# keio-bioinformatics/stem_kernel

Hardware: AMD Instinct MI355X
Metric: sequence-pairs/sec (Gram entries/s) at L=200 nt (higher is better)
Workload: dtype f64

## Files before the change

include/stem_kernel.h:

```cpp
#ifndef STEM_KERNEL_H
#define STEM_KERNEL_H

#include <stddef.h>
#include <stdint.h>

#ifdef __cplusplus
extern "C" {
#endif

#define SK_ABI_VERSION 3

typedef enum {
  SK_OK = 0,
  SK_ERR_INVALID = -1,
  SK_ERR_HIP = -2,
  SK_ERR_NO_DEVICE = -3,
  SK_ERR_ALLOC = -4,
  SK_ERR_RANGE = -5,
  SK_ERR_UNSUPPORTED = -6
} sk_status;

typedef enum {
  SK_SU_STEM = 0,
  SK_SI_STEM = 1,
  SK_SU_STR = 2,
  SK_SI_STR = 3,
  SK_SU_STEM_STR = 4,
  SK_SI_STEM_STR = 5,
  SK_LSU_STEM = 6,
  SK_LSU_STEM_STR = 7,
  SK_NAIVE_STR = 8,
  SK_BPLA = 9,
  SK_LA = 10,
  SK_BPLA_SW = 11,
  SK_LA_SW = 12,
  SK_STEM4D = 13,
  SK_AA_LA = 14,
  SK_AA_LA_SW = 15,
  SK_SIMPAL = 16
} sk_kernel_kind;

typedef struct {
  int32_t kind;
  uint32_t len_band;
  double beta;
  double loop_gap;
  double stack;
  double covar;
  double alpha;
  double gap;
  double match;
  double mismatch;
  double ext;
  double score_table[16];
  double subst;
  double bp_bound;
  int32_t bp_model;
  uint32_t loop;
  double ali_bound;
  int32_t ali_zerop_fixed;
  double aa_score_table[529];
} sk_kernel_params;

void sk_kernel_params_default(sk_kernel_params *p, int32_t kind);

typedef struct sk_context sk_context;

int sk_open(int device, void *hip_stream, sk_context **ctx);
int sk_close(sk_context *ctx);
const char *sk_strerror(int status);
const char *sk_last_error(const sk_context *ctx);

typedef struct sk_dataset sk_dataset;

int sk_dataset_create(sk_dataset **ds);
int sk_dataset_free(sk_dataset *ds);

int sk_dataset_add(sk_dataset *ds, const char *label, int n_rows,
                   const char *const *rows, const double *const *bpp_rows,
                   float th, int use_bp);
int sk_dataset_add_synthetic(sk_dataset *ds, int32_t n, const char *const *seqs,
                             const char *const *labels, float th, int32_t n_threads);
int sk_dataset_add_synthetic_rows(sk_dataset *ds, int32_t n, int32_t n_rows,
                                  const char *const *rows, const char *const *labels,
                                  float th, int32_t n_threads);
int sk_dataset_add_protein(sk_dataset *ds, const char *label, int n_rows,
                           const char *const *rows);
int sk_dataset_aa_profile(const sk_dataset *ds, int i, float *prof24, float *n_seqs);
int sk_char2aa(int c);
int sk_dataset_add_palindromes(sk_dataset *ds, const char *label, const char *seq,
                               const double *bpp, int32_t seed_length, int32_t min_loop,
                               int32_t max_dist);
int sk_dataset_add_palindrome_entries(sk_dataset *ds, const char *label, int32_t seed_length,
                                      int32_t n, const char *keys, const int32_t *dist,
                                      const float *weight);
int sk_dataset_palindromes(const sk_dataset *ds, int i, int32_t *n, char *keys, int32_t *dist,
                           float *weight);
int sk_simpal_shape(int32_t *y_tile, int32_t *x_block);
int sk_dataset_add_copy(sk_dataset *dst, const sk_dataset *src, int32_t i);
int sk_dataset_size(const sk_dataset *ds);
int sk_dataset_export(const sk_dataset *ds, int32_t first, int32_t count, uint8_t *buf,
                      size_t cap, size_t *size);
int sk_dataset_import(sk_dataset *ds, const uint8_t *buf, size_t size);
int sk_dataset_pack_digest(sk_dataset *ds, uint64_t *y_hash, uint64_t *x_hash);
const char *sk_dataset_label(const sk_dataset *ds, int i);
int sk_dataset_shape(const sk_dataset *ds, int i, int32_t *n_nodes,
                     int32_t *n_edges, int32_t *n_bpfreq, int32_t *n_roots,
                     int32_t *seq_len);
int sk_dataset_row_traffic(const sk_dataset *ds, int i, int32_t *rows, int32_t *stored,
                           int32_t *slab_reads, int32_t *gamma_reads, int32_t *phi_reads,
                           int32_t *reg_reads, int32_t *y_slots);
int sk_dataset_dag(const sk_dataset *ds, int i, uint32_t *first, uint32_t *last,
                   uint32_t *n_edges, uint32_t *n_bpfreq, float *weight,
                   uint32_t *max_pa, uint32_t *edge_to, uint32_t *edge_gaps,
                   uint32_t *bp_code, float *bp_p, uint32_t *roots,
                   float *pos_weight);

int sk_dataset_profile(const sk_dataset *ds, int i, float *prof5, float *n_seqs);

int sk_dataset_bpla_weights(const sk_dataset *ds, int i, float *p_left,
                            float *p_right, float *p_unpair);

int sk_dataset_upload(sk_context *ctx, sk_dataset *ds);

int sk_gram(sk_context *ctx, sk_dataset *ds, const sk_kernel_params *kp,
            int normalize, double *out);

int sk_pairs_device(sk_context *ctx, sk_dataset *ds, const sk_kernel_params *kp,
                    const int32_t *x, const int32_t *y, int64_t n_pairs,
                    double *out_dev);
int sk_pairs(sk_context *ctx, sk_dataset *ds, const sk_kernel_params *kp,
             const int32_t *x, const int32_t *y, int64_t n_pairs, double *out);

int sk_test_row(sk_context *ctx, sk_dataset *test, int t, sk_dataset *train,
                const int32_t *sv_index, int32_t n_sv,
                const sk_kernel_params *kp, double *out, double *self);

int sk_diagonal(sk_context *ctx, sk_dataset *ds, const int32_t *sv_index,
                int32_t n_sv, const sk_kernel_params *kp, double *out);

int sk_test_matrix(sk_context *ctx, sk_dataset *test, sk_dataset *train,
                   const sk_kernel_params *kp, int norm_test, int normalize,
                   double *out, double *self_out);

int64_t sk_shard_count(int32_t n, int32_t rank, int32_t world);
int sk_shard_cells(int32_t n, int32_t rank, int32_t world, int32_t *x, int32_t *y);
int sk_shard_assemble(int32_t n, int32_t world, const double *gathered, int64_t per_rank,
                      int normalize, double *out);
int sk_comm_unique_id(uint8_t *id, size_t id_bytes);
int sk_comm_init(sk_context *ctx, const uint8_t *id, size_t id_bytes, int32_t rank, int32_t world);
int sk_comm_allgather(sk_context *ctx, const double *send_dev, int64_t count, double *recv_dev);
int sk_gram_sharded(sk_context *ctx, sk_dataset *ds, const sk_kernel_params *kp, int normalize,
                    double *out);

int sk_format_libsvm(const double *matrix, int32_t rows, int32_t cols,
                     const char *const *labels, char *buf, size_t buf_size,
                     size_t *needed);

int sk_fold_synthetic(const char *seq, int32_t n, int32_t no_gu, double *out);

#define SK_FOLD_NO_GU 1
#define SK_FOLD_NO_CLOSING_GU 2
#define SK_FOLD_NO_LONELY_PAIRS 4
int sk_fold_mccaskill(sk_context *ctx, int32_t n, const char *const *seqs, int32_t flags,
                      double *out, double *log_z);
int sk_fold_sample(sk_context *ctx, int32_t n, const char *const *seqs, int32_t flags,
                   int32_t n_samples, uint64_t seed, double *out_bpp, char *out_structs,
                   double *log_z);
double sk_fold_sample_uniform(uint64_t seed, int32_t seq, int32_t sample, int32_t draw);
int sk_fold_alignment(sk_context *ctx, int32_t n_aln, const int32_t *n_rows,
                      const char *const *rows, int32_t flags, double *out, double *log_z);
int sk_dataset_add_consensus(sk_dataset *ds, const char *label, int n_rows,
                             const char *const *rows, const double *bpp, float th);
int sk_dataset_add_alifolded(sk_context *ctx, sk_dataset *ds, int32_t n, int32_t n_rows,
                             const char *const *rows, const char *const *labels, float th,
                             int32_t fold_flags, int32_t n_threads);
int sk_dataset_add_palindromes_folded(sk_context *ctx, sk_dataset *ds, int32_t n,
                                      const char *const *seqs, const char *const *labels,
                                      int32_t fold_flags, int32_t seed_length, int32_t min_loop,
                                      int32_t max_dist, int32_t n_threads);
int sk_dataset_add_batch(sk_dataset *ds, int32_t n, int32_t n_rows, const char *const *rows,
                         const double *const *bpp_rows, const char *const *labels, float th,
                         int32_t use_bp, int32_t n_threads);
int sk_dataset_add_folded(sk_context *ctx, sk_dataset *ds, int32_t n, int32_t n_rows,
                          const char *const *rows, const char *const *labels, float th,
                          int32_t fold_flags, int32_t n_threads);
int sk_dataset_add_sampled(sk_context *ctx, sk_dataset *ds, int32_t n, int32_t n_rows,
                           const char *const *rows, const char *const *labels, float th,
                           int32_t fold_flags, int32_t n_samples, uint64_t seed, int32_t n_threads);

int sk_bpla_gradients(sk_context *ctx, sk_dataset *xs, sk_dataset *ys, const sk_kernel_params *kp,
                      const int32_t *x, const int32_t *y, int64_t n_pairs, double *value,
                      double *grad);

typedef enum { SK_FMT_FASTA = 0, SK_FMT_CLUSTAL = 1, SK_FMT_MAF = 2 } sk_file_format;
typedef struct sk_seqfile sk_seqfile;
int sk_seqfile_read(const char *path, int32_t format, sk_seqfile **out);
int sk_seqfile_parse(const char *text, size_t len, int32_t format, sk_seqfile **out);
int sk_seqfile_free(sk_seqfile *f);
int64_t sk_seqfile_count(const sk_seqfile *f);
int32_t sk_seqfile_rows(const sk_seqfile *f, int64_t i);
const char *sk_seqfile_row(const sk_seqfile *f, int64_t i, int32_t r);
const char *sk_seqfile_last_error(void);
int sk_random_sequences(uint64_t *state, int32_t n_seqs, int32_t len, char *out);

typedef struct sk_svm_model sk_svm_model;
int sk_svm_model_load(const char *path, sk_svm_model **out);
void sk_svm_model_free(sk_svm_model *m);
int sk_svm_model_info(const sk_svm_model *m, int32_t *svm_type, int32_t *nr_class, int32_t *labels,
                      int32_t *has_probability);
int sk_svm_predict(const sk_svm_model *m, int32_t cnt, const double *row, int32_t n, int32_t probability,
                   double *label, double *values);
const char *sk_svm_last_error(void);

typedef struct {
  const int32_t *train;
  int32_t n_train;
  const int32_t *test;
  int32_t n_test;
  double Cp, Cn, eps;
  int64_t max_iter;
} sk_svm_problem;
typedef enum {
  SK_SVM_CONVERGED = 0,
  SK_SVM_NOT_CONVERGED = 1,
  SK_SVM_NO_PAIR = 2
} sk_svm_status;
typedef struct {
  double rho, obj;
  int64_t iterations;
  int32_t status;
  int32_t n_free;
  int32_t n_bound;
} sk_svm_solution;
int sk_svm_train_batch(sk_context *ctx, const double *gram, int32_t n, const double *labels,
                       const sk_svm_problem *problems, int32_t n_problems, double *alpha_out,
                       double *dec_out, sk_svm_solution *solutions);
int sk_svm_train_batch_host(const double *gram, int32_t n, const double *labels,
                            const sk_svm_problem *problems, int32_t n_problems, int32_t n_threads,
                            double *alpha_out, double *dec_out, sk_svm_solution *solutions);
typedef struct {
  int32_t shrink_calls;
  int32_t shrunk_calls;
  int32_t min_active;
  int32_t unshrunk;
  int32_t regrown;
  int32_t reconstructions;
  int32_t resumed;
} sk_svm_shrink_info;
int sk_svm_train_batch_ex(sk_context *ctx, const double *gram, int32_t n, const double *labels,
                          const sk_svm_problem *problems, int32_t n_problems, int32_t shrinking,
                          double *alpha_out, double *dec_out, sk_svm_solution *solutions,
                          sk_svm_shrink_info *info);
int sk_svm_train_batch_host_ex(const double *gram, int32_t n, const double *labels,
                               const sk_svm_problem *problems, int32_t n_problems, int32_t n_threads,
                               int32_t shrinking, double *alpha_out, double *dec_out,
                               sk_svm_solution *solutions, sk_svm_shrink_info *info);
int sk_svm_train_shape(int32_t *bounds, int32_t *n_classes, int32_t *max_train);
int sk_svm_model_write(const char *path, const double *labels, int32_t n, const int32_t *train,
                       int32_t n_train, const double *alpha, double rho);

typedef enum {
  SK_SVM_C_SVC = 0,
  SK_SVM_NU_SVC = 1,
// ... 102 lines not shown
```

stem_kernel_amd/_lib.py:

```python
from __future__ import annotations

import ctypes as C
import os
import threading

_HERE = os.path.dirname(os.path.abspath(__file__))
LIB_PATH = os.environ.get("SK_LIB_PATH") or os.path.join(_HERE, "libstem_kernel_amd.so")

SK_OK = 0
STATUS = {
    0: "ok", -1: "invalid argument", -2: "HIP runtime error", -3: "no usable gfx950 device",
    -4: "allocation failed", -5: "index out of range", -6: "unsupported",
}

FMT_FASTA, FMT_CLUSTAL, FMT_MAF = range(3)
(SU_STEM, SI_STEM, SU_STR, SI_STR, SU_STEM_STR, SI_STEM_STR, LSU_STEM, LSU_STEM_STR, NAIVE_STR,
 BPLA, LA, BPLA_SW, LA_SW, STEM4D, AA_LA, AA_LA_SW, SIMPAL) = range(17)
AA_LETTERS = "ARNDCQEGHILKMFPSTWYVBZX"


class KernelParams(C.Structure):
    _fields_ = [
        ("kind", C.c_int32), ("len_band", C.c_uint32), ("beta", C.c_double),
        ("loop_gap", C.c_double), ("stack", C.c_double), ("covar", C.c_double),
        ("alpha", C.c_double), ("gap", C.c_double), ("match", C.c_double),
        ("mismatch", C.c_double), ("ext", C.c_double), ("score_table", C.c_double * 16),
        ("subst", C.c_double), ("bp_bound", C.c_double), ("bp_model", C.c_int32),
        ("loop", C.c_uint32), ("ali_bound", C.c_double), ("ali_zerop_fixed", C.c_int32),
        ("aa_score_table", C.c_double * 529),
    ]


class SvmProblem(C.Structure):
    _fields_ = [("train", C.POINTER(C.c_int32)), ("n_train", C.c_int32), ("test", C.POINTER(C.c_int32)),
                ("n_test", C.c_int32), ("Cp", C.c_double), ("Cn", C.c_double), ("eps", C.c_double),
                ("max_iter", C.c_int64)]


class SvmSolution(C.Structure):
    _fields_ = [("rho", C.c_double), ("obj", C.c_double), ("iterations", C.c_int64), ("status", C.c_int32),
                ("n_free", C.c_int32), ("n_bound", C.c_int32)]


class AucProblem(C.Structure):
    _fields_ = [("train", C.POINTER(C.c_int32)), ("n_train", C.c_int32), ("test", C.POINTER(C.c_int32)),
                ("n_test", C.c_int32), ("C", C.c_double), ("alpha", C.POINTER(C.c_double)), ("rho", C.c_double),
                ("delta", C.POINTER(C.c_double))]


class SvmShrinkInfo(C.Structure):
    _fields_ = [(k, C.c_int32) for k in ("shrink_calls", "shrunk_calls", "min_active", "unshrunk", "regrown",
                                         "reconstructions", "resumed")]


class SvmTask(C.Structure):
    _fields_ = [("train", C.POINTER(C.c_int32)), ("n_train", C.c_int32), ("test", C.POINTER(C.c_int32)),
                ("n_test", C.c_int32), ("svm_type", C.c_int32), ("C", C.c_double), ("nu", C.c_double),
                ("p", C.c_double), ("eps", C.c_double), ("max_iter", C.c_int64)]


class SvmTaskSolution(C.Structure):
    _fields_ = [("rho", C.c_double), ("obj", C.c_double), ("iterations", C.c_int64), ("status", C.c_int32),
                ("n_free", C.c_int32), ("n_bound", C.c_int32), ("r", C.c_double)]


class AucInfo(C.Structure):
    _fields_ = [("n_free", C.c_int32), ("n_bound", C.c_int32), ("cg_iterations", C.c_int32),
                ("finite", C.c_int32)]


_P = C.c_void_p
_I32P = C.POINTER(C.c_int32)
_U32P = C.POINTER(C.c_uint32)
_F32P = C.POINTER(C.c_float)
_F64P = C.POINTER(C.c_double)
_I64P = C.POINTER(C.c_int64)

SIGNATURES = {
    "sk_kernel_params_default": (None, [C.POINTER(KernelParams), C.c_int32]),
    "sk_open": (C.c_int, [C.c_int, _P, C.POINTER(_P)]),
    "sk_close": (C.c_int, [_P]),
    "sk_strerror": (C.c_char_p, [C.c_int]),
    "sk_last_error": (C.c_char_p, [_P]),
    "sk_dataset_create": (C.c_int, [C.POINTER(_P)]),
    "sk_dataset_free": (C.c_int, [_P]),
    "sk_dataset_add": (C.c_int, [_P, C.c_char_p, C.c_int, C.POINTER(C.c_char_p),
                                 C.POINTER(_F64P), C.c_float, C.c_int]),
    "sk_dataset_add_synthetic": (C.c_int, [_P, C.c_int32, C.POINTER(C.c_char_p),
                                           C.POINTER(C.c_char_p), C.c_float, C.c_int32]),
    "sk_dataset_add_synthetic_rows": (C.c_int, [_P, C.c_int32, C.c_int32, C.POINTER(C.c_char_p),
                                                C.POINTER(C.c_char_p), C.c_float, C.c_int32]),
    "sk_dataset_add_protein": (C.c_int, [_P, C.c_char_p, C.c_int, C.POINTER(C.c_char_p)]),
    "sk_dataset_aa_profile": (C.c_int, [_P, C.c_int, _F32P, _F32P]),
    "sk_char2aa": (C.c_int, [C.c_int]),
    "sk_last_la_protein": (C.c_int, [_P, C.POINTER(C.c_uint32)]),
    "sk_dataset_add_palindromes": (C.c_int, [_P, C.c_char_p, C.c_char_p, C.POINTER(C.c_double),
                                             C.c_int32, C.c_int32, C.c_int32]),
    "sk_dataset_add_palindromes_folded": (C.c_int, [_P, _P, C.c_int32, C.POINTER(C.c_char_p),
                                                    C.POINTER(C.c_char_p), C.c_int32, C.c_int32,
                                                    C.c_int32, C.c_int32, C.c_int32]),
    "sk_dataset_add_palindrome_entries": (C.c_int, [_P, C.c_char_p, C.c_int32, C.c_int32, C.c_char_p,
                                                    C.POINTER(C.c_int32), _F32P]),
    "sk_dataset_palindromes": (C.c_int, [_P, C.c_int, C.POINTER(C.c_int32), C.c_char_p,
                                         C.POINTER(C.c_int32), _F32P]),
    "sk_simpal_shape": (C.c_int, [C.POINTER(C.c_int32), C.POINTER(C.c_int32)]),
    "sk_dataset_size": (C.c_int, [_P]),
    "sk_dataset_add_copy": (C.c_int, [_P, _P, C.c_int32]),
    "sk_dataset_export": (C.c_int, [_P, C.c_int32, C.c_int32, C.c_void_p, C.c_size_t,
                                    C.POINTER(C.c_size_t)]),
    "sk_dataset_import": (C.c_int, [_P, C.c_void_p, C.c_size_t]),
    "sk_dataset_pack_digest": (C.c_int, [_P, C.POINTER(C.c_uint64), C.POINTER(C.c_uint64)]),
    "sk_dataset_label": (C.c_char_p, [_P, C.c_int]),
    "sk_dataset_shape": (C.c_int, [_P, C.c_int, _I32P, _I32P, _I32P, _I32P, _I32P]),
    "sk_dataset_row_traffic": (C.c_int, [_P, C.c_int, _I32P, _I32P, _I32P, _I32P, _I32P, _I32P, _I32P]),
    "sk_dataset_dag": (C.c_int, [_P, C.c_int, _U32P, _U32P, _U32P, _U32P, _F32P, _U32P,
                                 _U32P, _U32P, _U32P, _F32P, _U32P, _F32P]),
    "sk_dataset_profile": (C.c_int, [_P, C.c_int, _F32P, _F32P]),
    "sk_dataset_bpla_weights": (C.c_int, [_P, C.c_int, _F32P, _F32P, _F32P]),
    "sk_dataset_upload": (C.c_int, [_P, _P]),
    "sk_gram": (C.c_int, [_P, _P, C.POINTER(KernelParams), C.c_int, _F64P]),
    "sk_pairs_device": (C.c_int, [_P, _P, C.POINTER(KernelParams), _I32P, _I32P, C.c_int64,
                                  C.c_void_p]),
    "sk_pairs": (C.c_int, [_P, _P, C.POINTER(KernelParams), _I32P, _I32P, C.c_int64, _F64P]),
    "sk_test_row": (C.c_int, [_P, _P, C.c_int, _P, _I32P, C.c_int32, C.POINTER(KernelParams),
                              _F64P, _F64P]),
    "sk_diagonal": (C.c_int, [_P, _P, _I32P, C.c_int32, C.POINTER(KernelParams), _F64P]),
    "sk_test_matrix": (C.c_int, [_P, _P, _P, C.POINTER(KernelParams), C.c_int, C.c_int, _F64P,
                                 _F64P]),
    "sk_format_libsvm": (C.c_int, [_F64P, C.c_int32, C.c_int32, C.POINTER(C.c_char_p),
                                   C.c_char_p, C.c_size_t, C.POINTER(C.c_size_t)]),
    "sk_fold_synthetic": (C.c_int, [C.c_char_p, C.c_int32, C.c_int32, _F64P]),
    "sk_fold_mccaskill": (C.c_int, [_P, C.c_int32, C.POINTER(C.c_char_p), C.c_int32, _F64P, _F64P]),
    "sk_fold_sample": (C.c_int, [_P, C.c_int32, C.POINTER(C.c_char_p), C.c_int32, C.c_int32, C.c_uint64,
                                 _F64P, C.c_void_p, _F64P]),
    "sk_fold_sample_uniform": (C.c_double, [C.c_uint64, C.c_int32, C.c_int32, C.c_int32]),
    "sk_fold_alignment": (C.c_int, [_P, C.c_int32, _I32P, C.POINTER(C.c_char_p), C.c_int32, _F64P, _F64P]),
    "sk_dataset_add_consensus": (C.c_int, [_P, C.c_char_p, C.c_int, C.POINTER(C.c_char_p), _F64P, C.c_float]),
    "sk_dataset_add_alifolded": (C.c_int, [_P, _P, C.c_int32, C.c_int32, C.POINTER(C.c_char_p),
                                           C.POINTER(C.c_char_p), C.c_float, C.c_int32, C.c_int32]),
    "sk_dataset_add_sampled": (C.c_int, [_P, _P, C.c_int32, C.c_int32, C.POINTER(C.c_char_p),
                                         C.POINTER(C.c_char_p), C.c_float, C.c_int32, C.c_int32,
                                         C.c_uint64, C.c_int32]),
    "sk_dataset_add_batch": (C.c_int, [_P, C.c_int32, C.c_int32, C.POINTER(C.c_char_p),
                                       C.POINTER(_F64P), C.POINTER(C.c_char_p), C.c_float,
                                       C.c_int32, C.c_int32]),
    "sk_dataset_add_folded": (C.c_int, [_P, _P, C.c_int32, C.c_int32, C.POINTER(C.c_char_p),
                                        C.POINTER(C.c_char_p), C.c_float, C.c_int32, C.c_int32]),
    "sk_random_sequences": (C.c_int, [C.POINTER(C.c_uint64), C.c_int32, C.c_int32, C.c_char_p]),
    "sk_last_timing": (C.c_int, [_P, _F64P, _F64P, _F64P, _I32P]),
    "sk_last_launch_ms": (C.c_int, [_P, _F64P, _I32P]),
    "sk_set_async": (C.c_int, [_P, C.c_int32]),
    "sk_sync_timing": (C.c_int, [_P]),
    "sk_shard_count": (C.c_int64, [C.c_int32, C.c_int32, C.c_int32]),
    "sk_shard_cells": (C.c_int, [C.c_int32, C.c_int32, C.c_int32, _I32P, _I32P]),
    "sk_shard_assemble": (C.c_int, [C.c_int32, C.c_int32, _F64P, C.c_int64, C.c_int, _F64P]),
    "sk_comm_unique_id": (C.c_int, [C.c_char_p, C.c_size_t]),
    "sk_comm_init": (C.c_int, [_P, C.c_char_p, C.c_size_t, C.c_int32, C.c_int32]),
    "sk_comm_allgather": (C.c_int, [_P, C.c_void_p, C.c_int64, C.c_void_p]),
    "sk_gram_sharded": (C.c_int, [_P, _P, C.POINTER(KernelParams), C.c_int, _F64P]),
    "sk_last_classes": (C.c_int, [_P, C.POINTER(C.c_uint32), C.POINTER(C.c_uint32)]),
    "sk_last_gamma_shared": (C.c_int32, [_P]),
    "sk_stem4d_col_shape": (C.c_int, [C.c_int32, C.c_int32, _I32P, _I32P, _I32P]),
    "sk_ribosum_tables": (None, [_F32P, _F32P]),
    "sk_char2rna": (C.c_int, [C.c_int]),
    "sk_experiments": (C.c_int, []),
    "sk_bpla_gradients": (C.c_int, [_P, _P, _P, C.POINTER(KernelParams), _I32P, _I32P, C.c_int64,
                                    _F64P, _F64P]),
    "sk_seqfile_read": (C.c_int, [C.c_char_p, C.c_int32, C.POINTER(_P)]),
    "sk_seqfile_parse": (C.c_int, [C.c_char_p, C.c_size_t, C.c_int32, C.POINTER(_P)]),
    "sk_seqfile_free": (C.c_int, [_P]),
    "sk_seqfile_count": (C.c_int64, [_P]),
    "sk_seqfile_rows": (C.c_int32, [_P, C.c_int64]),
    "sk_seqfile_row": (C.c_char_p, [_P, C.c_int64, C.c_int32]),
    "sk_seqfile_last_error": (C.c_char_p, []),
    "sk_svm_model_load": (C.c_int, [C.c_char_p, C.POINTER(_P)]),
    "sk_svm_model_free": (None, [_P]),
    "sk_svm_model_info": (C.c_int, [_P, C.POINTER(C.c_int32), C.POINTER(C.c_int32), C.POINTER(C.c_int32),
                                    C.POINTER(C.c_int32)]),
    "sk_svm_predict": (C.c_int, [_P, C.c_int32, C.POINTER(C.c_double), C.c_int32, C.c_int32,
                                 C.POINTER(C.c_double), C.POINTER(C.c_double)]),
    "sk_svm_last_error": (C.c_char_p, []),
    "sk_svm_train_batch": (C.c_int, [_P, _F64P, C.c_int32, _F64P, C.POINTER(SvmProblem), C.c_int32, _F64P, _F64P,
                                     C.POINTER(SvmSolution)]),
    "sk_svm_train_batch_host": (C.c_int, [_F64P, C.c_int32, _F64P, C.POINTER(SvmProblem), C.c_int32, C.c_int32,
                                          _F64P, _F64P, C.POINTER(SvmSolution)]),
    "sk_svm_train_batch_ex": (C.c_int, [_P, _F64P, C.c_int32, _F64P, C.POINTER(SvmProblem), C.c_int32, C.c_int32,
                                        _F64P, _F64P, C.POINTER(SvmSolution), C.POINTER(SvmShrinkInfo)]),
    "sk_svm_train_batch_host_ex": (C.c_int, [_F64P, C.c_int32, _F64P, C.POINTER(SvmProblem), C.c_int32, C.c_int32,
                                             C.c_int32, _F64P, _F64P, C.POINTER(SvmSolution),
                                             C.POINTER(SvmShrinkInfo)]),
    "sk_svm_train_shape": (C.c_int, [_I32P, _I32P, _I32P]),
    "sk_svm_model_write": (C.c_int, [C.c_char_p, _F64P, C.c_int32, _I32P, C.c_int32, _F64P, C.c_double]),
    "sk_svm_solve_batch": (C.c_int, [_P, _F64P, C.c_int32, _F64P, C.POINTER(SvmTask), C.c_int32, _F64P, _F64P,
                                     C.POINTER(SvmTaskSolution)]),
    "sk_svm_solve_batch_host": (C.c_int, [_F64P, C.c_int32, _F64P, C.POINTER(SvmTask), C.c_int32, C.c_int32,
                                          _F64P, _F64P, C.POINTER(SvmTaskSolution)]),
    "sk_svm_solve_shape": (C.c_int, [_I32P]),
    "sk_svm_model_write_ex": (C.c_int, [C.c_char_p, C.c_int32, _F64P, C.c_int32, _I32P, C.c_int32, _F64P,
                                        C.c_double]),
    "sk_auc_delta": (C.c_int, [_F64P, _F64P, C.c_int32, _F64P, _F64P]),
    "sk_auc_gradient_batch": (C.c_int, [_P, _F64P, _F64P, C.c_int32, C.c_int32, _F64P, C.POINTER(AucProblem),
                                        C.c_int32, _F64P, _F64P, _F64P, C.POINTER(AucInfo)]),
    "sk_auc_gradient_batch_host": (C.c_int, [_F64P, _F64P, C.c_int32, C.c_int32, _F64P, C.POINTER(AucProblem),
                                             C.c_int32, C.c_int32, _F64P, _F64P, _F64P, C.POINTER(AucInfo)]),
    "sk_auc_gradient_shape": (C.c_int, [_I32P, _I32P, C.POINTER(C.c_int64)]),
    "sk_features_create": (C.c_int, [C.c_int32, _I64P, _I32P, _F64P, _I32P, C.POINTER(_P)]),
    "sk_features_parse": (C.c_int, [C.c_char_p, C.c_size_t, C.POINTER(_P)]),
    "sk_features_read": (C.c_int, [C.c_char_p, C.POINTER(_P)]),
    "sk_features_free": (C.c_int, [_P]),
    "sk_features_shape": (C.c_int, [_P, _I32P, _I32P, _I64P]),
    "sk_features_labels": (C.c_int, [_P, _I32P]),
    "sk_features_rows": (C.c_int, [_P, _I64P, _I32P, _F64P]),
    "sk_features_last_error": (C.c_char_p, []),
    "sk_feature_gram_shape": (C.c_int, [_I32P, _I32P, _I32P, _I64P]),
    "sk_feature_dots": (C.c_int, [_P, _P, _P, _F64P]),
    "sk_feature_dots_host": (C.c_int, [_P, _P, C.c_int32, _F64P]),
    "sk_feature_gram": (C.c_int, [_P, _P, C.c_int32, C.c_int32, _F64P, _F64P, _F64P]),
    "sk_feature_gram_host": (C.c_int, [_P, C.c_int32, C.c_int32, _F64P, C.c_int32, _F64P, _F64P]),
    "sk_feature_gram_cross": (C.c_int, [_P, _P, _P, C.c_int32, C.c_int32, _F64P, _F64P]),
    "sk_feature_gram_cross_host": (C.c_int, [_P, _P, C.c_int32, C.c_int32, _F64P, C.c_int32, _F64P]),
}

_lock = threading.Lock()
_lib = None


class StemKernelError(RuntimeError):

    def __init__(self, code, msg=""):
        super().__init__(f"{STATUS.get(code, code)}{': ' + msg if msg else ''}")
        self.code = code


def lib():
    global _lib
    with _lock:
        if _lib is not None:
            return _lib
        if not os.path.exists(LIB_PATH):
            raise StemKernelError(-3, f"{LIB_PATH} not built; run `make` or __graft_entry__.build()")
        try:
            import torch
        except Exception:
            pass
        L = C.CDLL(LIB_PATH)
        for name, (res, args) in SIGNATURES.items():
            f = getattr(L, name)
            f.restype = res
            f.argtypes = args
        _lib = L
        return L


def check(rc, ctx=None):
    if rc != SK_OK:
        msg = ""
        if ctx:
            m = lib().sk_last_error(ctx)
            msg = m.decode() if m else ""
        raise StemKernelError(rc, msg)
    return rc


def default_params(kind=SU_STEM_STR, **over):
    p = KernelParams()
    lib().sk_kernel_params_default(C.byref(p), kind)
    for k, v in over.items():
# ... 8 lines not shown
```

stem_kernel_amd/csrc/host/dataset.cpp:

```cpp
#include <hip/hip_runtime.h>

#include <algorithm>
#include <atomic>
#include <cctype>
#include <chrono>
#include <cmath>
#include <cstdio>
#include <cstdlib>
#include <cstring>
#include <map>
#include <new>
#include <string>
#include <thread>
#include <utility>
#include <vector>

#include "host/runtime_types.h"
#include "blosum62.inc"

namespace sk {
namespace {
int pal_code(char c) {
  switch (c) {
    case 'a': return 0;
// ... 266 lines not shown
    };
    std::vector<Ent> v((size_t)n);
    for (int32_t k = 0; k < n; ++k) {
      uint64_t key = 0;
      for (int t = 0; t < seed_length; ++t) {
        const int c = sk::pal_code(keys[(size_t)k * seed_length + t]);
        if (c < 0) {
          ds->err = "palindrome key letter outside acgu";
          return SK_ERR_INVALID;
        }
        key = (key << 2) | (uint64_t)c;
      }
      if (dist[k] < 0 || !(weight[k] >= 0.0f) || !std::isfinite(weight[k])) {
        ds->err = "palindrome entry with a negative dist or a weight that is not finite and non-negative";
        return SK_ERR_INVALID;
      }
      v[(size_t)k] = Ent{key, dist[k], weight[k]};
    }
    std::sort(v.begin(), v.end(),
              [](const Ent& a, const Ent& b) { return a.key != b.key ? a.key < b.key : a.dist < b.dist; });
    for (size_t k = 1; k < v.size(); ++k)
      if (v[k].key == v[k - 1].key && v[k].dist == v[k - 1].dist) {
        ds->err = "duplicate palindrome entry (key, dist)";
        return SK_ERR_INVALID;
      }
    sk::Example ex;
    ex.pal = true;
    ex.pal_seed = seed_length;
    ex.n_rows = 1;
    ex.n_seqs = 1.0f;
    ex.rows.assign(1, std::string());
    for (const Ent& e : v) {
      ex.pal_key.push_back(e.key);
      ex.pal_dist.push_back(e.dist);
      ex.pal_w.push_back(e.w);
    }
    ds->ex.push_back(std::move(ex));
    ds->labels.emplace_back(label ? label : "");
  } catch (const std::bad_alloc&) {
    return SK_ERR_ALLOC;
  }
  return SK_OK;
}

int sk_dataset_palindromes(const sk_dataset* ds, int i, int32_t* n, char* keys, int32_t* dist, float* weight) {
  if (!ds) return SK_ERR_INVALID;
  if (i < 0 || i >= (int)ds->ex.size()) return SK_ERR_RANGE;
  const sk::Example& X = ds->ex[i];
  if (!X.pal) return SK_ERR_INVALID;
  const size_t m = X.pal_key.size();
  if (n) *n = (int32_t)m;
  if (keys)
    for (size_t k = 0; k < m; ++k)
      for (int t = 0; t < X.pal_seed; ++t)
        keys[k * X.pal_seed + t] = "acgu"[(X.pal_key[k] >> (2 * (X.pal_seed - 1 - t))) & 3];
  if (dist) std::copy(X.pal_dist.begin(), X.pal_dist.end(), dist);
  if (weight) std::copy(X.pal_w.begin(), X.pal_w.end(), weight);
  return SK_OK;
}

int sk_dataset_add_synthetic_rows(sk_dataset* ds, int32_t n, int32_t n_rows,
                                  const char* const* rows, const char* const* labels, float th,
                                  int32_t n_threads) {
  if (!ds || n < 0 || n_rows < 1 || (n > 0 && !rows)) return SK_ERR_INVALID;
  if (ds->uploaded || sk::ds_mixes(ds, sk::kSortRna)) return SK_ERR_INVALID;
  const size_t base = ds->ex.size();
  try {
    ds->ex.resize(base + n);
    for (int32_t i = 0; i < n; ++i) ds->labels.emplace_back(labels && labels[i] ? labels[i] : "+1");
  } catch (const std::bad_alloc&) {
    return SK_ERR_ALLOC;
  }
  int nt = n_threads > 0 ? n_threads : (int)std::thread::hardware_concurrency();
  nt = std::max(1, std::min(nt, std::max<int32_t>(n, 1)));
  std::atomic<int32_t> next(0), status(SK_OK);
  static const bool stats = std::getenv("SK_HOST_STATS") != nullptr;
  std::atomic<int64_t> ns_fold(0), ns_build(0);
  auto work = [&]() {
    std::vector<std::vector<double>> bpp(n_rows);
    std::vector<const double*> bptr(n_rows);
    for (;;) {
      const int32_t i = next.fetch_add(1);
      if (i >= n || status.load() != SK_OK) return;
      try {
        const auto t0 = std::chrono::steady_clock::now();
        const char* const* ex_rows = rows + (size_t)i * n_rows;
        for (int32_t r = 0; r < n_rows; ++r) {
          const char* s = ex_rows[r];
          const int L = (int)std::strlen(s);
          std::string row;
          for (int k = 0; k < L; ++k)
            if (s[k] != '-') row.push_back((char)std::tolower((unsigned char)s[k]));
          bpp[r].assign(row.size() > 1 ? row.size() * (row.size() - 1) / 2 : 1, 0.0);
          sk::fold_nussinov(row.c_str(), (int)row.size(), false, bpp[r].data());
          bptr[r] = bpp[r].data();
        }
        const auto t1 = std::chrono::steady_clock::now();
        sk::build_example(ds->ex[base + i], n_rows, ex_rows, bptr.data(), th, true);
        if (stats) {
          const auto t2 = std::chrono::steady_clock::now();
          ns_fold += std::chrono::duration_cast<std::chrono::nanoseconds>(t1 - t0).count();
          ns_build += std::chrono::duration_cast<std::chrono::nanoseconds>(t2 - t1).count();
        }
      } catch (...) {
        status.store(SK_ERR_INVALID);
      }
    }
  };
  sk::run_pool(nt, work);
  if (stats)
    std::fprintf(stderr, "[sk] synthetic examples: %d on %d threads, fold %.3f s, build %.3f s (thread-seconds)\n", n,
                 nt, ns_fold.load() * 1e-9, ns_build.load() * 1e-9);
  if (status.load() != SK_OK) {
    ds->ex.resize(base);
    ds->labels.resize(base);
  }
  return status.load();
}

int sk_dataset_add_synthetic(sk_dataset* ds, int32_t n, const char* const* seqs,
                             const char* const* labels, float th, int32_t n_threads) {
  return sk_dataset_add_synthetic_rows(ds, n, 1, seqs, labels, th, n_threads);
}

int sk_dataset_size(const sk_dataset* ds) { return ds ? (int)ds->ex.size() : 0; }

const char* sk_dataset_label(const sk_dataset* ds, int i) {
  if (!ds || i < 0 || i >= (int)ds->labels.size()) return nullptr;
  return ds->labels[i].c_str();
}

int sk_dataset_shape(const sk_dataset* ds, int i, int32_t* n_nodes, int32_t* n_edges,
                     int32_t* n_bpfreq, int32_t* n_roots, int32_t* seq_len) {
  if (!ds) return SK_ERR_INVALID;
  if (i < 0 || i >= (int)ds->ex.size()) return SK_ERR_RANGE;
  const sk::Example& X = ds->ex[i];
  if (n_nodes) *n_nodes = X.n_nodes();
  if (n_edges) *n_edges = X.n_edges();
  if (n_bpfreq) *n_bpfreq = (int32_t)X.bpf_code.size();
  if (n_roots) *n_roots = (int32_t)X.roots.size();
  if (seq_len) *seq_len = X.len;
  return SK_OK;
}

int sk_dataset_row_traffic(const sk_dataset* ds, int i, int32_t* rows, int32_t* stored,
                           int32_t* slab_reads, int32_t* gamma_reads, int32_t* phi_reads,
                           int32_t* reg_reads, int32_t* y_slots) {
  if (!ds) return SK_ERR_INVALID;
  if (i < 0 || i >= (int)ds->ex.size()) return SK_ERR_RANGE;
  const sk::HostPack& P = ds->pack;
  if ((int)P.ex_nlxg.size() != (int)ds->ex.size()) return SK_ERR_INVALID;
  int32_t st = 0, sl = 0, ga = 0, ph = 0, rg = 0;
  uint32_t prev = 0xffffu;
  size_t k = (size_t)P.ex_xgch_base[i];
  for (size_t r = (size_t)P.ex_xg_base[i]; r < (size_t)P.ex_xg_base[i] + P.ex_nlxg[i]; ++r) {
    const int ne = P.xgrow[r].a & 0xff;
    for (int t = 0; t < ne; ++t, ++k) {
      const uint32_t c = P.xg_ch[k] & 0xffffu;
      if (c == prev) ++rg;
      else if (c & 0x8000u) ++ga;
      else if (c & 0x4000u) ++ph;
      else ++sl;
    }
    prev = P.xgrow[r].b >> 16;
    st += prev < 0x4000u;
  }
  if (rows) *rows = P.ex_nlxg[i];
  if (stored) *stored = st;
  if (slab_reads) *slab_reads = sl;
  if (gamma_reads) *gamma_reads = ga;
  if (phi_reads) *phi_reads = ph;
  if (reg_reads) *reg_reads = rg;
  if (y_slots) *y_slots = P.ex_nl[i];
  return SK_OK;
}

int sk_dataset_dag(const sk_dataset* ds, int i, uint32_t* first, uint32_t* last,
                   uint32_t* n_edges, uint32_t* n_bpfreq, float* weight, uint32_t* max_pa,
                   uint32_t* edge_to, uint32_t* edge_gaps, uint32_t* bp_code, float* bp_p,
                   uint32_t* roots, float* pos_weight) {
  if (!ds) return SK_ERR_INVALID;
  if (i < 0 || i >= (int)ds->ex.size()) return SK_ERR_RANGE;
  const sk::Example& X = ds->ex[i];
  const int n = X.n_nodes();
  for (int v = 0; v < n; ++v) {
    if (first) first[v] = X.first[v];
    if (last) last[v] = X.last[v];
    if (n_edges) n_edges[v] = X.edge_off[v + 1] - X.edge_off[v];
    if (n_bpfreq) n_bpfreq[v] = X.bpf_off[v + 1] - X.bpf_off[v];
    if (weight) weight[v] = X.weight[v];
    if (max_pa) max_pa[v] = X.max_pa[v];
  }
  if (edge_to) std::copy(X.edge_to.begin(), X.edge_to.end(), edge_to);
  if (edge_gaps) std::copy(X.edge_gaps.begin(), X.edge_gaps.end(), edge_gaps);
  if (bp_code) std::copy(X.bpf_code.begin(), X.bpf_code.end(), bp_code);
  if (bp_p) std::copy(X.bpf_p.begin(), X.bpf_p.end(), bp_p);
  if (roots) std::copy(X.roots.begin(), X.roots.end(), roots);
  if (pos_weight && X.has_bp) std::copy(X.pos_weight.begin(), X.pos_weight.end(), pos_weight);
  return SK_OK;
}

int sk_dataset_profile(const sk_dataset* ds, int i, float* prof5, float* n_seqs) {
  if (!ds) return SK_ERR_INVALID;
  if (i < 0 || i >= (int)ds->ex.size()) return SK_ERR_RANGE;
  const sk::Example& X = ds->ex[i];
  if (prof5) std::copy(X.prof5.begin(), X.prof5.end(), prof5);
  if (n_seqs) *n_seqs = X.n_seqs;
  return SK_OK;
}

int sk_dataset_bpla_weights(const sk_dataset* ds, int i, float* p_left, float* p_right,
                            float* p_unpair) {
  if (!ds) return SK_ERR_INVALID;
  if (i < 0 || i >= (int)ds->ex.size()) return SK_ERR_RANGE;
  const sk::Example& X = ds->ex[i];
  for (int k = 0; k < X.len; ++k) {
    const float4 w = sk::bpla_weight(X, k);
    if (p_left) p_left[k] = w.x;
    if (p_right) p_right[k] = w.y;
    if (p_unpair) p_unpair[k] = w.z;
  }
  return SK_OK;
}

int sk_dataset_add_batch(sk_dataset* ds, int32_t n, int32_t n_rows, const char* const* rows,
                         const double* const* bpp_rows, const char* const* labels, float th,
                         int32_t use_bp, int32_t n_threads) {
  if (!ds || n < 0 || n_rows < 1 || (n > 0 && (!rows || (use_bp && !bpp_rows)))) return SK_ERR_INVALID;
  if (ds->uploaded) return SK_ERR_INVALID;
  return sk::add_examples_threaded(ds, n, n_rows, rows, bpp_rows, labels, th, use_bp, n_threads);
}

}
```

stem_kernel_amd/csrc/host/pack.cpp:

```cpp
#include <hip/hip_runtime.h>

#include <algorithm>
#include <atomic>
#include <chrono>
#include <cmath>
#include <cstdio>
#include <cstdlib>
#include <cstring>
#include <functional>
#include <numeric>
#include <queue>
#include <string>
#include <thread>
#include <type_traits>
#include <utility>
#include <vector>

#include "host/runtime_types.h"

namespace sk {
namespace {

void bpla_weights(const Example& X, std::vector<float4>& out) {
  const int L = X.len;
  const size_t base = out.size();
  out.resize(base + (size_t)std::max(L, 0));
  if (!X.has_bp) {
    for (int i = 0; i < L; ++i) out[base + i] = make_float4(0.f, 0.f, 1.f, 0.f);
    return;
  }
  std::vector<float> pr((size_t)L, 0.0f);
  for (int i = 0; i < L; ++i) {
    float pl = 0.0f;
    if (i + 1 < L) {
      const double* row = X.bpp.data() + sk::tri_index(L, i, i + 1);
      for (int j = i + 1; j < L; ++j) {
        const double b = row[j - i - 1];
        pl = (float)((double)pl + b);
        pr[j] = (float)((double)pr[j] + b);
      }
    }
    float pu = (float)(1.0 - (double)(pl + pr[i]));
    if (pu < 0.0f) pu = 0.0f;
    out[base + i] = make_float4(std::sqrt(pl), std::sqrt(pr[i]), std::sqrt(pu), 0.f);
  }
}

static void pack_palindromes(sk_dataset* ds) {
  sk_dataset::PalPack& P = ds->spack;
  P = sk_dataset::PalPack();
  P.ex_off.push_back(0);
  for (const Example& X : ds->ex) {
    P.key.insert(P.key.end(), X.pal_key.begin(), X.pal_key.end());
    P.dist.insert(P.dist.end(), X.pal_dist.begin(), X.pal_dist.end());
    P.w.insert(P.w.end(), X.pal_w.begin(), X.pal_w.end());
    P.ex_off.push_back((int32_t)P.key.size());
  }
}

static void pack_protein(sk_dataset* ds) {
  sk_dataset::ProtPack& P = ds->ppack;
  P = sk_dataset::ProtPack();
  size_t pos = 0;
  for (const Example& X : ds->ex) pos += (size_t)X.len;
  P.prof.reserve(pos * sk::kAaSlots);
  P.code.reserve(pos);
  for (const Example& X : ds->ex) {
    P.ex_len.push_back(X.len);
    P.ex_pos_base.push_back((int32_t)P.code.size());
    bool coded = true;
    for (int i = 0; i < X.len; ++i) {
      const float* c = X.aa_prof.data() + (size_t)i * sk::kAaSlots;
      int used = 0, slot = sk::kAaSlots - 1;
      for (int k = 0; k < sk::kAaSlots; ++k)
        if (c[k] != 0.0f) {
          ++used;
          slot = k;
        }
      coded = coded && used == 1;
      P.code.push_back((uint8_t)slot);
    }
    if (!coded) std::fill(P.code.end() - X.len, P.code.end(), (uint8_t)(sk::kAaSlots - 1));
    P.ex_coded.push_back(coded ? 1 : 0);
    P.prof.insert(P.prof.end(), X.aa_prof.begin(), X.aa_prof.end());
  }
}

static void assign_sweep_lanes(const std::vector<int>& take, const std::vector<uint32_t>& er, int nl,
                               uint32_t lanes[64]) {
  const int n = (int)take.size();
  thread_local uint8_t npar[2048];
  int cntp[64];
  for (int i = 0; i < n; ++i) ++npar[(er[take[i]] >> 11) & 0x7ff];
  for (int i = 0; i < n; ++i) cntp[i] = npar[(er[take[i]] >> 11) & 0x7ff];
  for (int i = 0; i < n; ++i) npar[(er[take[i]] >> 11) & 0x7ff] = 0;
  int ord[64];
  {
    int cstart[66] = {0};
    for (int i = 0; i < n; ++i) ++cstart[64 - cntp[i] + 1];
    for (int k = 0; k < 65; ++k) cstart[k + 1] += cstart[k];
    for (int i = 0; i < n; ++i) ord[cstart[64 - cntp[i]]++] = i;
  }
  int fill[4] = {0, 0, 0, 0};
  int at[4][16];
  uint32_t rd[2][32][4];
  int rdn[2][32];
  std::memset(at, 0, sizeof(at));
  std::memset(rdn, 0, sizeof(rdn));
  auto child_load = [&](int h, uint32_t c) {
    const int sl = c & 31;
    for (int t = 0; t < std::min(rdn[h][sl], 4); ++t)
      if (rd[h][sl][t] == c) return rdn[h][sl];
    return rdn[h][sl] + 1;
  };
  auto put = [&](int g, uint32_t r) {
    const uint32_t c = r & 0x7ff, q = (r >> 11) & 0x7ff;
    const int h = g >> 1, sl = c & 31;
    bool seen = false;
    for (int t = 0; t < std::min(rdn[h][sl], 4); ++t) seen |= rd[h][sl][t] == c;
    if (!seen) {
      if (rdn[h][sl] < 4) rd[h][sl][rdn[h][sl]] = c;
      ++rdn[h][sl];
    }
    at[g][q & 15]++;
    lanes[16 * g + fill[g]++] = r;
  };
  for (int oi = 0; oi < n; ++oi) {
    const int i = ord[oi];
    const uint32_t r = er[take[i]];
    const uint32_t c = r & 0x7ff, q = (r >> 11) & 0x7ff;
    int best = -1, bc = 1 << 30;
    for (int g = 0; g < 4; ++g) {
      if (fill[g] == 16) continue;
      const int cost = 4 * (child_load(g >> 1, c) + at[g][q & 15] + 1) + fill[g];
      if (cost < bc) {
        bc = cost;
        best = g;
      }
    }
    put(best, r);
  }
  const int nl1 = std::max(nl, 1);
  for (int g = 0; g < 4; ++g) {
    while (fill[g] < 16) {
      int bs = 0, bc = 1 << 30;
      for (int sl = 0; sl < 32 && sl < nl1; ++sl) {
        const int cost = rdn[g >> 1][sl] + at[g][sl & 15];
        if (cost < bc) {
          bc = cost;
          bs = sl;
        }
      }
      const uint32_t d = (uint32_t)(bs % nl1);
      put(g, d | (d << 11));
    }
  }
}

bool is_gamma(const Example& X, int v) {
  const uint32_t e0 = X.edge_off[v], e1 = X.edge_off[v + 1];
  if (e1 - e0 != 1) return false;
  const uint32_t c = X.edge_to[e0];
  if (X.edge_off[c + 1] != X.edge_off[c]) return false;
  return X.bpf_off[v + 1] - X.bpf_off[v] == 1 && X.prof5[(size_t)X.first[v] * 5 + 4] == 0.0f;
}
uint32_t gamma_key(const Example& X, int v) {
  return ((uint32_t)X.bpf_code[X.bpf_off[v]] << 16) | (uint32_t)(X.last[v] - X.first[v]);
}
bool is_phi(const Example& X, int v) {
  const uint32_t e0 = X.edge_off[v], e1 = X.edge_off[v + 1];
  if (e1 == e0 || 2 * (e1 - e0) + 1 > 255) return false;
  if (X.bpf_off[v + 1] - X.bpf_off[v] != 1 || X.prof5[(size_t)X.first[v] * 5 + 4] != 0.0f) return false;
  for (uint32_t k = e0; k < e1; ++k)
    if (!is_gamma(X, X.edge_to[k])) return false;
  return !is_gamma(X, v);
}

struct KeyTables {
  std::vector<uint32_t> gam_key;
  std::vector<uint64_t> phi_raw;
  bool gam_on = false, phi_on = false;
  uint32_t gamma_idx(uint32_t key) const {
    return (uint32_t)(std::lower_bound(gam_key.begin(), gam_key.end(), key) - gam_key.begin());
  }
  uint32_t phi_idx(uint32_t key_p, uint32_t key_c) const {
    const uint64_t k = ((uint64_t)key_c << 32) | key_p;
    return (uint32_t)(std::lower_bound(phi_raw.begin(), phi_raw.end(), k) - phi_raw.begin());
  }
};

KeyTables key_tables(const std::vector<Example>& ex, int nthr) {
  KeyTables K;
  const int n = (int)ex.size();
  {
    std::vector<std::vector<uint32_t>> tk(nthr);
    std::vector<std::vector<uint64_t>> tp(nthr);
    auto keys = [&](int t) {
      for (int e = (int)((int64_t)n * t / nthr); e < (int)((int64_t)n * (t + 1) / nthr); ++e) {
        const Example& X = ex[e];
        for (int v = 0; v < X.n_nodes(); ++v) {
          if (is_gamma(X, v)) tk[t].push_back(gamma_key(X, v));
          if (is_phi(X, v)) {
            tk[t].push_back(gamma_key(X, v));
            for (uint32_t k = X.edge_off[v]; k < X.edge_off[v + 1]; ++k)
              tp[t].push_back(((uint64_t)gamma_key(X, X.edge_to[k]) << 32) | gamma_key(X, v));
          }
        }
        auto& k1 = tk[t];
        if (k1.size() > 4096) {
          std::sort(k1.begin(), k1.end());
          k1.erase(std::unique(k1.begin(), k1.end()), k1.end());
        }
        auto& p1 = tp[t];
        if (p1.size() > 4096) {
          std::sort(p1.begin(), p1.end());
          p1.erase(std::unique(p1.begin(), p1.end()), p1.end());
        }
      }
    };
    run_slices(nthr, keys);
    for (int t = 0; t < nthr; ++t) {
      K.gam_key.insert(K.gam_key.end(), tk[t].begin(), tk[t].end());
      K.phi_raw.insert(K.phi_raw.end(), tp[t].begin(), tp[t].end());
    }
  }
  std::sort(K.gam_key.begin(), K.gam_key.end());
  K.gam_key.erase(std::unique(K.gam_key.begin(), K.gam_key.end()), K.gam_key.end());
  K.gam_on = !K.gam_key.empty() && K.gam_key.size() <= 512 && !SK_KNOB("SK_NO_GAMMA");
  if (!K.gam_on) K.gam_key.clear();
  std::sort(K.phi_raw.begin(), K.phi_raw.end());
  K.phi_raw.erase(std::unique(K.phi_raw.begin(), K.phi_raw.end()), K.phi_raw.end());
  K.phi_on = K.gam_on && !K.phi_raw.empty() && K.phi_raw.size() < 0x4000 && !SK_KNOB("SK_NO_PHI");
  return K;
}

struct YJob {
  int nb0, ebase, bbase, nl;
  bool big;
};
struct YOut {
  std::vector<uint32_t> ysc, ye2, yn_a, yn_b, yn_c;
  std::vector<int32_t> ycs;
  std::vector<uint4> yrec;
  std::vector<float> yn_w, yn_nbp, yn_p0;
  std::vector<double> yn_P;
  int nch = 0;
  std::string err;
};
void pack_y(const HostPack& P, bool sweep_lanes_greedy, const YJob& J, YOut& Y) {
  const int nl = J.nl, ebase = J.ebase, bbase = J.bbase;
  const bool big = J.big;
  {
    std::vector<int> srt(nl);
    std::iota(srt.begin(), srt.end(), 0);
    auto len_of = [&](int k) { return P.nd_b[J.nb0 + k] & 0xffff; };
    std::stable_sort(srt.begin(), srt.end(), [&](int a, int b) { return len_of(a) < len_of(b); });
    std::vector<int> pos(nl);
    for (int i = 0; i < nl; ++i) pos[srt[i]] = i;
    const int nb0 = J.nb0;
    if (big) {
      const int lmax = nl ? (int)(P.nd_b[nb0 + srt[nl - 1]] & 0xffff) : 0;
      for (int v = 0; v <= lmax + 1; ++v) Y.ycs.push_back(0);
      Y.nch = 0;
    } else {
      std::vector<uint32_t> er;
      std::vector<int> epar, ech;
      for (int k = 0; k < nl; ++k) {
        const uint32_t a = P.nd_a[nb0 + k];
        const uint32_t ne = (a >> 16) & 0xff, el = a & 0xffff;
        for (uint32_t t = 0; t < ne; ++t) {
          const uint2 rec = P.ed[ebase + el + t];
          const int c = pos[rec.x & 0xffff], q = pos[k];
          epar.push_back(q);
          ech.push_back(c);
          er.push_back((uint32_t)c | ((uint32_t)q << 11) | ((rec.x >> 16) << 22));
        }
      }
      const int ne_all = (int)er.size();
      std::vector<int> cb(nl + 1, 0), by_child(ne_all);
      for (int f = 0; f < ne_all; ++f) cb[ech[f] + 1]++;
      for (int i = 0; i < nl; ++i) cb[i + 1] += cb[i];
      {
        std::vector<int> fillc(cb.begin(), cb.end() - 1);
        for (int f = 0; f < ne_all; ++f) by_child[fillc[ech[f]]++] = f;
      }
      std::vector<int> h(nl, 0), rem(nl, 0);
      for (int i = nl - 1; i >= 0; --i)
        for (int t = cb[i]; t < cb[i + 1]; ++t) h[i] = std::max(h[i], h[epar[by_child[t]]] + 1);
      for (int f = 0; f < ne_all; ++f) rem[epar[f]]++;
      std::priority_queue<uint64_t, std::vector<uint64_t>, std::greater<uint64_t>> ready;
      auto push_edges_of = [&](int c) {
        const uint64_t len = P.nd_b[nb0 + srt[c]] & 0xffff;
        for (int t = cb[c]; t < cb[c + 1]; ++t) {
          const int f = by_child[t];
          ready.push(((uint64_t)((1 << 20) - 1 - h[epar[f]]) << 44) | (len << 28) | (uint64_t)f);
        }
      };
      for (int c = 0; c < nl; ++c)
        if (rem[c] == 0) push_edges_of(c);
      std::vector<int32_t> cm;
      int32_t run = -1, placed = 0;
      std::vector<int> take, done;
      while (!ready.empty()) {
        take.clear();
        done.clear();
        while (!ready.empty() && (int)take.size() < 64) {
          take.push_back((int)(ready.top() & 0xfffffffu));
          ready.pop();
        }
        for (int f : take) {
          run = std::max<int32_t>(run, (int32_t)(P.nd_b[nb0 + srt[ech[f]]] & 0xffff));
          if (--rem[epar[f]] == 0) done.push_back(epar[f]);
        }
        if (sweep_lanes_greedy) {
          uint32_t lanes[64];
          assign_sweep_lanes(take, er, nl, lanes);
          Y.ysc.insert(Y.ysc.end(), lanes, lanes + 64);
        } else {
          for (int f : take) Y.ysc.push_back(er[f]);
          for (int j = (int)take.size(); j < 64; ++j) {
            const uint32_t d = (uint32_t)(j % std::max(nl, 1));
            Y.ysc.push_back(d | (d << 11));
          }
        }
        placed += (int)take.size();
        cm.push_back(run);
        for (int q : done) push_edges_of(q);
      }
      if (placed != ne_all) {
        Y.err = "IY sweep schedule: DAG has a cycle";
        return;
      }
      const int nch = (int)cm.size();
      const int lmax = nl ? (int)(P.nd_b[nb0 + srt[nl - 1]] & 0xffff) : 0;
      for (int v = 0, c = 0; v <= lmax + 1; ++v) {
        while (c < nch && cm[c] < v) ++c;
        Y.ycs.push_back(c);
      }
      Y.nch = nch;
    }
    const int ye2_base = (int)Y.ye2.size();
    for (int i = 0; i < nl; ++i) {
      const int k = srt[i];
      const uint32_t a = P.nd_a[nb0 + k];
      const uint32_t ne = (a >> 16) & 0xff, el = a & 0xffff;
      const uint32_t nbf = a >> 24, bl = P.nd_b[nb0 + k] >> 16;
      Y.yn_a.push_back(((uint32_t)Y.ye2.size() - ye2_base) | (a & 0xffff0000u));
      for (uint32_t t = 0; t < ne; ++t) {
        const uint2 rec = P.ed[ebase + el + t];
        Y.ye2.push_back(big ? 0u : (uint32_t)pos[rec.x & 0xffff] | ((uint32_t)i << 11) |
                                       ((rec.x >> 16) << 22));
      }
      const bool one = nbf == 1 && P.nd_nbp[nb0 + k] == 0.0f;
      const uint32_t bc0 = nbf ? P.bpf_code[bbase + bl] & 0xf : 0u;
      Y.yn_c.push_back((P.nd_c[nb0 + k] & 0xffff) | (bc0 << 16) | ((one ? 1u : 0u) << 24));
      Y.yn_p0.push_back(nbf ? P.bpf_p[bbase + bl] : 0.0f);
      {
        uint4 r;
        r.x = Y.yn_a.back();
        r.y = Y.yn_c.back();
        std::memcpy(&r.z, &P.nd_w[nb0 + k], 4);
        std::memcpy(&r.w, &Y.yn_p0.back(), 4);
        Y.yrec.push_back(r);
      }
      Y.yn_b.push_back(P.nd_b[nb0 + k]);
      Y.yn_w.push_back(P.nd_w[nb0 + k]);
      Y.yn_nbp.push_back(P.nd_nbp[nb0 + k]);
      Y.yn_P.push_back(P.nd_P[nb0 + k]);
    }
  }
}

struct XOut {
  std::vector<uint32_t> nd_a, nd_b, nd_c, xr_ch, xr_node, gr_info, xg_ch, xg_clg, phk_idx, gra_gidx,
      gra_row, xg_node;
  std::vector<float> nd_w, nd_nbp, bpf_p, gr_pf, xg_cpf, ex_nseqs, pos_w;
  std::vector<double> nd_P, gr_P;
  std::vector<uint2> ed;
  std::vector<uint32_t> bpf_code;
  std::vector<int32_t> lvl, ex_nslots, ex_nlxg, ex_gapless, ex_nl, ex_nlev, ex_len, ex_has_w;
  std::vector<uint8_t> ex_big, xg_cty, pos_chr, ex_dyadic, ex_str_fast, ex_onehot;
  std::vector<sk::XRow> xrow, xgrow;
  std::vector<float4> pos_prof, pos_lru;
  std::vector<uint64_t> ex_phi_bits;
  int nl = 0, nlev = 0, max_slots = 0, n_nostore = 0, n_nodes = 0, gslots = 0;
  bool big = false;
  int rc = SK_OK;
  std::string err;
};
void pack_x(const Example& X, const KeyTables& K, XOut& O) {
  const int nn = X.n_nodes();
  std::vector<int> level(nn, -1);
  int nlev = 0;
  for (int v = 0; v < nn; ++v) {
    const uint32_t e0 = X.edge_off[v], e1 = X.edge_off[v + 1];
    if (e0 == e1) continue;
    int lv = 0;
    bool any_leaf = false;
    for (uint32_t k = e0; k < e1; ++k) {
      const int c = level[X.edge_to[k]];
      if (c < 0) any_leaf = true;
      else lv = std::max(lv, c + 1);
    }
    if (any_leaf && e1 - e0 != 1) {
      O.err = "unexpected DAG shape: stem with a leaf child";
      O.rc = SK_ERR_INVALID;
      return;
    }
    level[v] = lv;
    nlev = std::max(nlev, lv + 1);
  }
  std::vector<int> order;
  {
    std::vector<int> lstart(nlev + 1, 0);
    for (int v = 0; v < nn; ++v)
      if (level[v] >= 0) ++lstart[level[v] + 1];
    for (int l = 0; l < nlev; ++l) lstart[l + 1] += lstart[l];
    order.resize(lstart[nlev]);
    for (int v = 0; v < nn; ++v)
      if (level[v] >= 0) order[lstart[level[v]]++] = v;
  }
  const int nl = (int)order.size();
  if (nl >= 0xffff) {
    O.err = "example too large: more than 65534 non-leaf DAG nodes";
    O.rc = SK_ERR_UNSUPPORTED;
    return;
  }
  std::vector<int> nid(nn, -1);
  for (int k = 0; k < nl; ++k) nid[order[k]] = k;
  std::vector<uint8_t> fl(nn, 0);
  std::vector<uint32_t> gix(nn, 0);
  if (K.gam_on)
    for (int v = 0; v < nn; ++v) fl[v] |= is_gamma(X, v) ? 1 : 0;
  if (K.phi_on)
    for (int v = 0; v < nn; ++v) fl[v] |= is_phi(X, v) ? 2 : 0;
  for (int v = 0; v < nn; ++v)
    if (fl[v]) gix[v] = K.gamma_idx(gamma_key(X, v));
  {
    const size_t ne_x = (size_t)X.n_edges();
    for (auto* q : {&O.nd_a, &O.nd_b, &O.nd_c, &O.xr_node, &O.xg_node}) q->reserve(nl);
    O.nd_w.reserve(nl);
    O.nd_nbp.reserve(nl);
    O.nd_P.reserve(nl);
    O.ed.reserve(ne_x);
    O.xr_ch.reserve(ne_x);
    O.xrow.reserve(nl);
    O.xgrow.reserve(nl);
    O.xg_ch.reserve(2 * ne_x + nl);
    O.xg_clg.reserve(2 * ne_x + nl);
    O.xg_cpf.reserve(2 * ne_x + nl);
    O.xg_cty.reserve(2 * ne_x + nl);
    O.bpf_code.reserve(X.bpf_off[nn]);
    O.bpf_p.reserve(X.bpf_off[nn]);
  }
  std::vector<double> Pw(nn, 0.0);
  for (uint32_t r : X.roots) Pw[r] += 1.0;
  for (int v = nn - 1; v >= 0; --v)
    for (uint32_t k = X.edge_off[v]; k < X.edge_off[v + 1]; ++k) Pw[X.edge_to[k]] += Pw[v];


  bool big_gap = false;
  for (int k = 0; k < nl; ++k) {
    const int v = order[k];
    const uint32_t e0 = X.edge_off[v], e1 = X.edge_off[v + 1];
    const uint32_t b0 = X.bpf_off[v], b1 = X.bpf_off[v + 1];
    const bool loop = level[v] == 0;
    const uint32_t eloc = (uint32_t)O.ed.size(), bloc = (uint32_t)O.bpf_code.size();
    const uint32_t ne = loop ? 0u : e1 - e0;
    if (eloc > 0xffff || bloc > 0xffff || ne > 0xff || b1 - b0 > 0xff ||
        X.last[v] - X.first[v] > 0xffff) {
      O.err = "example too large for the 16-bit packed DAG layout";
      O.rc = SK_ERR_UNSUPPORTED;
      return;
    }
    O.nd_a.push_back(eloc | (ne << 16) | ((b1 - b0) << 24));
    O.nd_b.push_back((X.last[v] - X.first[v]) | (bloc << 16));
    O.nd_c.push_back(loop ? X.edge_gaps[e0] : 0u);
    O.nd_w.push_back(X.weight[v]);
    O.nd_nbp.push_back(X.prof5[(size_t)X.first[v] * 5 + 4]);
    O.nd_P.push_back(Pw[v]);
    if (!loop) {
      for (uint32_t t = e0; t < e1; ++t) {
        const int c = nid[X.edge_to[t]];
        if (c < 0 || X.edge_gaps[t] > 0xffff) {
          O.err = c < 0 ? "unexpected DAG shape: stem with a leaf child" : "gap count exceeds 65535";
          O.rc = c < 0 ? SK_ERR_INVALID : SK_ERR_UNSUPPORTED;
          return;
        }
        big_gap |= X.edge_gaps[t] > 1023;
        O.ed.push_back(make_uint2((uint32_t)c | (X.edge_gaps[t] << 16), (uint32_t)k));
      }
    }
    for (uint32_t t = b0; t < b1; ++t) {
      O.bpf_code.push_back(X.bpf_code[t]);
      O.bpf_p.push_back(X.bpf_p[t]);
    }
  }
  std::vector<int32_t> lv(nlev + 1, 0);
  for (int k = 0; k < nl; ++k) lv[level[order[k]] + 1]++;
  for (int l = 0; l < nlev; ++l) lv[l + 1] += lv[l];
  O.lvl.insert(O.lvl.end(), lv.begin(), lv.end());
  const bool big = nl > 2047 || big_gap;
  O.ex_big.push_back(big ? 1 : 0);

  O.nl = nl;
  O.big = big;

  {
    std::vector<int> last_parent(nn, -1);
    for (int v = 0; v < nn; ++v)
      for (uint32_t k = X.edge_off[v]; k < X.edge_off[v + 1]; ++k)
        last_parent[X.edge_to[k]] = std::max(last_parent[X.edge_to[k]], v);
    std::vector<uint32_t> slot(nn, 0xffff);
    std::vector<int> free_list;
    int nslots = 0;
    for (int v = 0; v < nn; ++v) {
      if (level[v] < 0) continue;
      const bool loop = level[v] == 0;
      const uint32_t e0 = X.edge_off[v], e1 = X.edge_off[v + 1];
      const uint32_t b0 = X.bpf_off[v], b1 = X.bpf_off[v + 1];
      uint32_t nch = 0;
      if (!loop) {
        for (uint32_t k = e0; k < e1; ++k) {
          const int c = X.edge_to[k];
          O.xr_ch.push_back(slot[c] | (X.edge_gaps[k] << 16));
          ++nch;
        }
      }
      for (uint32_t k = e0; k < e1; ++k) {
        const int c = X.edge_to[k];
        if (level[c] >= 0 && last_parent[c] == v && slot[c] != 0xffff) free_list.push_back(slot[c]);
      }
      if (last_parent[v] >= 0) {
        int sl;
        if (!free_list.empty()) {
          sl = free_list.back();
          free_list.pop_back();
        } else {
          sl = nslots++;
        }
        slot[v] = (uint32_t)sl;
      }
      sk::XRow xr;
      xr.a = nch | ((b1 - b0) << 8) | ((loop ? X.edge_gaps[e0] : 0u) << 16);
      xr.b = (X.last[v] - X.first[v]) | (slot[v] << 16);
      xr.w = X.weight[v];
      xr.nbp = X.prof5[(size_t)X.first[v] * 5 + 4];
      xr.bp0 = b1 > b0 ? X.bpf_p[b0] : 0.0f;
      xr.P = Pw[v];
      xr.c = (O.nd_b[nid[v]] >> 16) | ((b1 > b0 ? (uint32_t)X.bpf_code[b0] : 0u) << 16);
      O.xrow.push_back(xr);
      O.xr_node.push_back((uint32_t)nid[v]);
    }
    if (nslots >= 0xffff) {
      O.err = "too many live DAG rows";
      O.rc = SK_ERR_UNSUPPORTED;
      return;
    }
    O.ex_nslots.push_back(nslots);
    O.max_slots = std::max(O.max_slots, nslots);

    std::vector<uint32_t> gslot(nn, 0xffff);
    std::vector<int> gfree;
    int gslots = 0, nlxg = 0;
    std::vector<int> order;
    {
      std::vector<int> npar(nn, 0), cand(nn, -1);
      for (int v = 0; v < nn; ++v)
        for (uint32_t k = X.edge_off[v]; k < X.edge_off[v + 1]; ++k) ++npar[X.edge_to[k]];
      for (int v = 0; v < nn; ++v) {
        if (level[v] <= 0 || (fl[v] & 2)) continue;
        for (uint32_t k = X.edge_off[v]; k < X.edge_off[v + 1] && k < X.edge_off[v] + 4; ++k) {
          const int c = X.edge_to[k];
          if (npar[c] == 1 && level[c] >= 0 && !(fl[c] & 1)) {
            cand[v] = c;
            break;
          }
        }
      }
      if (SK_KNOB("SK_REF_ORDER")) {
        for (int v = 0; v < nn; ++v)
          if (level[v] >= 0) order.push_back(v);
      } else {
        std::vector<uint8_t> seen(nn, 0);
        std::vector<std::pair<int, int>> st;
        auto dfs = [&](int s) {
          if (seen[s] || level[s] < 0) return;
          seen[s] = 1;
          st.push_back({s, 0});
          while (!st.empty()) {
            auto& [v, i] = st.back();
            const int ne = (int)(X.edge_off[v + 1] - X.edge_off[v]);
            int next = -1;
            while (i >= 0 && i < ne && next < 0) {
              const int c = X.edge_to[X.edge_off[v] + i++];
              if (c != cand[v] && !seen[c] && level[c] >= 0) next = c;
            }
            if (next < 0 && i >= 0) {
              i = -1;
              if (cand[v] >= 0 && !seen[cand[v]]) next = cand[v];
            }
            if (next < 0) {
              order.push_back(v);
              st.pop_back();
            } else {
              seen[next] = 1;
              st.push_back({next, 0});
            }
          }
        };
        for (uint32_t r : X.roots) dfs((int)r);
        for (int v = nn - 1; v >= 0; --v) dfs(v);
      }
      std::vector<int> pos(nn, nn), first_parent(nn, nn);
      for (int i = 0; i < (int)order.size(); ++i) pos[order[i]] = i;
      for (int v = 0; v < nn; ++v)
        for (uint32_t k = X.edge_off[v]; k < X.edge_off[v + 1]; ++k) {
          const int c = X.edge_to[k];
          if (pos[v] < nn && (first_parent[c] == nn || pos[v] < pos[first_parent[c]])) first_parent[c] = v;
        }
      const bool move = K.phi_on && !SK_KNOB("SK_PHI_POSTORDER");
      std::vector<int> o1, boff(nn + 2, 0), bl;
      o1.reserve(order.size());
      for (int v : order) {
        if (move && (fl[v] & 2)) ++boff[first_parent[v] + 1];
        else o1.push_back(v);
      }
      for (int i = 0; i <= nn; ++i) boff[i + 1] += boff[i];
      bl.resize(boff[nn + 1]);
      {
        std::vector<int> bf(boff.begin(), boff.end() - 1);
        for (int v : order)
          if (move && (fl[v] & 2)) bl[bf[first_parent[v]]++] = v;
      }
      std::vector<int> o2;
      o2.reserve(order.size() + 8);
      for (int v : o1) {
        const auto bb = bl.begin() + boff[v], be = bl.begin() + boff[v + 1];
        const auto it = std::find(bb, be, cand[v]);
        if (it != be) {
          std::rotate(it, it + 1, be);
          o2.insert(o2.end(), bb, be);
        } else if (bb != be && cand[v] >= 0 && !o2.empty() && o2.back() == cand[v]) {
          o2.pop_back();
          o2.insert(o2.end(), bb, be);
          o2.push_back(cand[v]);
        } else {
          o2.insert(o2.end(), bb, be);
        }
        o2.push_back(v);
      }
      o2.insert(o2.end(), bl.begin() + boff[nn], bl.begin() + boff[nn + 1]);
      order.swap(o2);
    }
    std::vector<int> glast(nn, -1);
    {
      std::vector<int> gpos(nn, -1);
      for (int i = 0; i < (int)order.size(); ++i) gpos[order[i]] = i;
      for (int v : order)
        for (uint32_t k = X.edge_off[v]; k < X.edge_off[v + 1]; ++k) {
          const int c = X.edge_to[k];
          if (glast[c] < 0 || gpos[v] > gpos[glast[c]]) glast[c] = v;
        }
    }
    std::vector<uint8_t> nostore(nn, 0);
    if (!SK_KNOB("SK_STORE_ALL")) {
      std::vector<int> npar(nn, 0), emitted;
      for (int v = 0; v < nn; ++v)
        for (uint32_t k = X.edge_off[v]; k < X.edge_off[v + 1]; ++k) ++npar[X.edge_to[k]];
      for (int v : order)
        if (!(fl[v] & 1)) emitted.push_back(v);
      for (size_t i = 0; i + 1 < emitted.size(); ++i) {
        const int v = emitted[i], r = emitted[i + 1];
        if (npar[v] != 1 || level[r] <= 0 || level[v] < 0 || (fl[r] & 2)) continue;
        for (uint32_t k = X.edge_off[r]; k < X.edge_off[r + 1] && k < X.edge_off[r] + 4; ++k)
          if (X.edge_to[k] == v) nostore[v] = 1;
      }
    }
    for (int v : order) {
      const uint32_t e0 = X.edge_off[v], e1 = X.edge_off[v + 1];
      const uint32_t b0 = X.bpf_off[v], b1 = X.bpf_off[v + 1];
      if (fl[v] & 1) {
        O.gr_info.push_back(gix[v] | (X.edge_gaps[e0] << 16));
        O.gr_pf.push_back(X.bpf_p[b0]);
        O.gr_P.push_back(Pw[v]);
        continue;
      }
      const bool loop = level[v] == 0;
      const bool phi = (fl[v] & 2) != 0;
      uint32_t nch = 0;
      if (phi) {
        const uint32_t kp = gamma_key(X, v);
        for (uint32_t k = e0; k < e1; ++k) {
          const int c = X.edge_to[k];
          const uint32_t kc = gamma_key(X, c);
          const uint32_t pi = K.phi_idx(kp, kc);
          for (int ty : {2, 4}) {
            O.xg_ch.push_back(((ty == 2 ? 0x4000u | pi : 0x8000u | gix[c])) | (X.edge_gaps[k] << 16));
            O.xg_clg.push_back(X.edge_gaps[X.edge_off[c]]);
            O.xg_cpf.push_back(X.bpf_p[X.bpf_off[c]]);
            O.xg_cty.push_back((uint8_t)ty);
          }
          O.phk_idx.push_back(pi);
        }
        O.xg_ch.push_back(0x8000u | gix[v]);
        O.xg_clg.push_back(0u);
        O.xg_cpf.push_back(0.0f);
        O.xg_cty.push_back(3);
        O.gra_gidx.push_back(gix[v]);
        O.gra_row.push_back((uint32_t)O.xgrow.size());
        nch = 2 * (e1 - e0) + 1;
      } else if (!loop) {
        for (uint32_t k = e0; k < e1; ++k) {
          const int c = X.edge_to[k];
          if (fl[c] & 1) {
            O.xg_ch.push_back((0x8000u | gix[c]) | (X.edge_gaps[k] << 16));
            O.xg_clg.push_back(X.edge_gaps[X.edge_off[c]]);
            O.xg_cpf.push_back(X.bpf_p[X.bpf_off[c]]);
            O.xg_cty.push_back(1);
          } else {
            O.xg_ch.push_back(gslot[c] | (X.edge_gaps[k] << 16));
            O.xg_clg.push_back(0u);
            O.xg_cpf.push_back(1.0f);
            O.xg_cty.push_back(0);
          }
          ++nch;
        }
      }
      for (uint32_t k = e0; k < e1; ++k) {
        const int c = X.edge_to[k];
        if (level[c] >= 0 && glast[c] == v && gslot[c] < 0x4000) {
          gfree.push_back(gslot[c]);
          gslot[c] |= 0x10000;
        }
      }
      if (nostore[v]) {
        gslot[v] = 0xfffe;
      } else if (last_parent[v] >= 0) {
        int sl;
        if (!gfree.empty()) {
          sl = gfree.back();
          gfree.pop_back();
        } else {
          sl = gslots++;
        }
        gslot[v] = (uint32_t)sl;
      }
      sk::XRow xr;
      xr.a = nch | ((b1 - b0) << 8) | ((loop ? X.edge_gaps[e0] : 0u) << 16);
      xr.b = (X.last[v] - X.first[v]) | (gslot[v] << 16);
      xr.w = X.weight[v];
      xr.nbp = X.prof5[(size_t)X.first[v] * 5 + 4];
      xr.bp0 = b1 > b0 ? X.bpf_p[b0] : 0.0f;
      xr.P = Pw[v];
      xr.c = (O.nd_b[nid[v]] >> 16) | ((b1 > b0 ? (uint32_t)X.bpf_code[b0] : 0u) << 16) |
             (phi ? 0x80000000u : 0u);
      O.xgrow.push_back(xr);
      O.xg_node.push_back((uint32_t)nid[v]);
      ++nlxg;
    }
    if (K.phi_on) {
      const size_t W = (K.phi_raw.size() + 63) / 64;
      O.ex_phi_bits.assign(W, 0ull);
      for (size_t j = 0; j < O.phk_idx.size(); ++j)
        O.ex_phi_bits[O.phk_idx[j] / 64] |= 1ull << (O.phk_idx[j] % 64);
    }
    if (gslots >= 0x4000) {
      O.err = "too many live DAG rows";
      O.rc = SK_ERR_UNSUPPORTED;
      return;
    }
    O.ex_nlxg.push_back(nlxg);
    O.max_slots = std::max(O.max_slots, gslots);
    O.n_nostore = 0;
    for (int v = 0; v < nn; ++v) O.n_nostore += nostore[v];
    O.n_nodes = nn;
    O.gslots = gslots;
  }
  {
    bool gl = true;
    for (int k = 0; k < nl; ++k) gl &= O.nd_nbp[k] == 0.0f;
    O.ex_gapless.push_back(gl ? 1 : 0);
  }
  O.ex_nl.push_back(nl);
  O.ex_nlev.push_back(nlev);
  O.nlev = nlev;
  O.ex_nseqs.push_back(X.n_seqs);
  O.ex_len.push_back(X.len);
  O.ex_has_w.push_back(X.has_bp ? 1 : 0);
  for (int i = 0; i < X.len; ++i) {
    const float* c = &X.prof5[(size_t)i * 5];
    O.pos_prof.push_back(make_float4(c[0], c[1], c[2], c[3]));
    O.pos_w.push_back(X.has_bp ? X.pos_weight[i] : 1.0f);
    O.pos_chr.push_back((uint8_t)X.rows[0][i]);
  }
  bpla_weights(X, O.pos_lru);
  {
    bool dy = true;
    for (int i = 0; i < X.len; ++i)
      for (int k = 0; k < 4; ++k) {
        const float v = X.prof5[(size_t)i * 5 + k] * 256.0f;
        dy = dy && v == std::rint(v);
      }
    O.ex_dyadic.push_back(dy ? 1 : 0);
    bool full = true;
    for (int i = 0; i < X.len; ++i) {
      const float* c = &X.prof5[(size_t)i * 5];
      full = full && (c[0] + c[1] + c[2] + c[3]) > 0.0f;
    }
    O.ex_str_fast.push_back(dy && full ? 1 : 0);
    bool oh = true;
    for (int i = 0; i < X.len && oh; ++i) {
      const float* c = &X.prof5[(size_t)i * 5];
      int ones = 0, zeros = 0;
      for (int k = 0; k < 4; ++k) {
        ones += c[k] == 1.0f;
        zeros += c[k] == 0.0f;
      }
      oh = ones == 1 && zeros == 3;
    }
    O.ex_onehot.push_back(oh ? 1 : 0);
  }
}

}

float4 bpla_weight(const Example& X, int i) {
  if (!X.has_bp) return make_float4(0.f, 0.f, 1.f, 0.f);
  float pl = 0.0f, pr = 0.0f;
  for (int j = 0; j < i; ++j) pr = (float)((double)pr + X.bpp[sk::tri_index(X.len, j, i)]);
  for (int j = i + 1; j < X.len; ++j) pl = (float)((double)pl + X.bpp[sk::tri_index(X.len, i, j)]);
  float pu = (float)(1.0 - (double)(pl + pr));
  if (pu < 0.0f) pu = 0.0f;
  return make_float4(std::sqrt(pl), std::sqrt(pr), std::sqrt(pu), 0.f);
}

int pack_dataset(sk_dataset* ds, std::string& err, const std::function<void()>* after_x) {
  HostPack& P = ds->pack;
  const bool tstats = std::getenv("SK_HOST_STATS") != nullptr;
  auto tnow = [] { return std::chrono::duration<double, std::milli>(std::chrono::steady_clock::now().time_since_epoch()).count(); };
  const double tp0 = tnow();
  const char* lanes_env = SK_KNOB("SK_SWEEP_LANES");
  const bool sweep_lanes_greedy = !lanes_env || std::atoi(lanes_env) != 0;
  P = HostPack();
  const int n = (int)ds->ex.size();
  const size_t pcap = std::getenv("SK_PACK_THREADS") ? (size_t)std::max(1, std::atoi(std::getenv("SK_PACK_THREADS")))
                                                     : (size_t)16;
  const int nthr = (int)std::max<size_t>(1, std::min<size_t>({(size_t)n / 8 + 1, pcap,
                                                              (size_t)std::max(1u, std::thread::hardware_concurrency())}));
  const KeyTables K = key_tables(ds->ex, nthr);
  P.gam_key = K.gam_key;
  if (K.phi_on)
    for (uint64_t k : K.phi_raw) {
      P.phi_al.push_back((uint32_t)k);
      P.phi_g.push_back(K.gamma_idx((uint32_t)(k >> 32)));
    }
  std::vector<YJob> yjobs;
  yjobs.reserve(n);
  const double tp1 = tnow();
  double tpx = tp1;
  {
    std::vector<XOut> xo(n);
    std::atomic<int> next{0};
    auto work = [&]() {
      for (int e = next.fetch_add(1); e < n; e = next.fetch_add(1)) pack_x(ds->ex[e], K, xo[e]);
    };
    run_pool(nthr, work);
    tpx = tnow();
    P.ex_node_base.push_back(0);
    P.ex_edge_base.push_back(0);
    P.ex_bpf_base.push_back(0);
    P.ex_lvl_base.push_back(0);
    P.ex_pos_base.push_back(0);
#define SK_BIG(X) X(nd_a) X(nd_b) X(nd_c) X(nd_w) X(nd_nbp) X(nd_P) X(ed) X(bpf_code) X(bpf_p) X(lvl) \
  X(xr_ch) X(xrow) X(xr_node) X(gr_info) X(gr_pf) X(gr_P) X(xg_ch) X(xg_clg) X(xg_cpf) X(xg_cty)    \
  X(phk_idx) X(gra_gidx) X(gra_row) X(xgrow) X(xg_node) X(pos_prof) X(pos_w) X(pos_chr) X(pos_lru)  \
  X(ex_phi_bits)
#define SK_OFF(f) std::vector<size_t> off_##f(n + 1, 0);
    SK_BIG(SK_OFF)
#undef SK_OFF
    auto app = [](auto& dst, const auto& src) { dst.insert(dst.end(), src.begin(), src.end()); };
    std::vector<long> st_nodes(n), st_nost(n), st_slots(n);
    for (int e = 0; e < n; ++e) {
      XOut& O = xo[e];
      st_nodes[e] = O.n_nodes;
      st_nost[e] = O.n_nostore;
      st_slots[e] = O.gslots;
      if (O.rc) {
        err = O.err;
        return O.rc;
      }
#define SK_ACC(f) off_##f[e + 1] = off_##f[e] + O.f.size();
      SK_BIG(SK_ACC)
#undef SK_ACC
      yjobs.push_back(YJob{(int)off_nd_a[e], (int)off_ed[e], (int)off_bpf_code[e], O.nl, O.big});
      P.ex_xch_base.push_back((int32_t)off_xr_ch[e]);
      P.ex_xg_base.push_back((int32_t)off_xgrow[e]);
      P.ex_xgch_base.push_back((int32_t)off_xg_ch[e]);
      P.ex_gr_base.push_back((int32_t)off_gr_info[e]);
      P.ex_gra_base.push_back((int32_t)off_gra_gidx[e]);
      P.ex_phk_base.push_back((int32_t)off_phk_idx[e]);
      app(P.ex_big, O.ex_big); app(P.ex_nslots, O.ex_nslots); app(P.ex_nlxg, O.ex_nlxg);
      app(P.ex_gapless, O.ex_gapless); app(P.ex_nl, O.ex_nl); app(P.ex_nlev, O.ex_nlev);
      app(P.ex_nseqs, O.ex_nseqs); app(P.ex_len, O.ex_len); app(P.ex_has_w, O.ex_has_w);
      app(P.ex_dyadic, O.ex_dyadic); app(P.ex_str_fast, O.ex_str_fast); app(P.ex_onehot, O.ex_onehot);
      P.max_slots = std::max(P.max_slots, O.max_slots);
      P.ex_node_base.push_back((int32_t)off_nd_a[e + 1]);
      P.ex_edge_base.push_back((int32_t)off_ed[e + 1]);
      P.ex_bpf_base.push_back((int32_t)off_bpf_code[e + 1]);
      P.ex_lvl_base.push_back((int32_t)off_lvl[e + 1]);
      P.ex_pos_base.push_back((int32_t)off_pos_prof[e + 1]);
      P.max_nl = std::max(P.max_nl, O.nl);
      P.max_edges = std::max(P.max_edges, (int)O.ed.size());
      P.max_bpf = std::max(P.max_bpf, (int)O.bpf_code.size());
      P.max_nlev = std::max(P.max_nlev, O.nlev);
      P.max_len = std::max(P.max_len, ds->ex[e].len);
    }
    const double tq1 = tnow();
#define SK_SIZE(f) P.f.resize(off_##f[n]);
    SK_BIG(SK_SIZE)
#undef SK_SIZE
    const double tq2 = tnow();
    {
      std::atomic<int> nx{0};
      auto copy = [&]() {
        for (int e = nx.fetch_add(1); e < n; e = nx.fetch_add(1)) {
          XOut& O = xo[e];
          for (uint32_t& r : O.gra_row) r += (uint32_t)off_xgrow[e];
#define SK_CPY(f) std::copy(O.f.begin(), O.f.end(), P.f.begin() + off_##f[e]);
          SK_BIG(SK_CPY)
#undef SK_CPY
          O = XOut();
        }
      };
      run_pool(nthr, copy);
    }
    if (tstats) fprintf(stderr, "[sk pack] offsets %.1f ms, resize %.1f ms, copy %.1f ms\n", tq1 - tpx, tq2 - tq1, tnow() - tq2);
#undef SK_BIG
    if (tstats) fprintf(stderr, "[sk pack] keys %.1f ms, x-role %.1f ms (%d threads) + append %.1f ms\n",
                        tp1 - tp0, tpx - tp1, nthr, tnow() - tpx);
    if (std::getenv("SK_PACK_STATS")) {
      long s_rows = 0, s_nost = 0, s_slots = 0, s_nodes = 0, s_st = 0, s_slab = 0, s_gam = 0, s_phi = 0,
           s_reg = 0;
      for (int e = 0; e < n; ++e) {
        s_rows += P.ex_nlxg[e];
        s_nodes += st_nodes[e];
        s_nost += st_nost[e];
        s_slots += st_slots[e];
        uint32_t prev = 0xffffu;
        size_t k = (size_t)P.ex_xgch_base[e];
        for (size_t r = (size_t)P.ex_xg_base[e]; r < (size_t)P.ex_xg_base[e] + P.ex_nlxg[e]; ++r) {
          const int ne = P.xgrow[r].a & 0xff;
          for (int t = 0; t < ne; ++t, ++k) {
            const uint32_t c = P.xg_ch[k] & 0xffffu;
            if (c == prev) ++s_reg;
            else if (c & 0x8000u) ++s_gam;
            else if (c & 0x4000u) ++s_phi;
            else ++s_slab;
          }
          prev = P.xgrow[r].b >> 16;
          s_st += prev < 0x4000u;
        }
      }
      fprintf(stderr,
              "[sk pack] gamma schedule: %ld nodes, %ld rows, %ld unstored, %ld slots; stored %ld, reads: "
              "slab %ld gamma %ld phi %ld, from registers %ld\n",
              s_nodes, s_rows, s_nost, s_slots, s_st, s_slab, s_gam, s_phi, s_reg);
    }
  }
  if (after_x) (*after_x)();
  const double tp2 = tnow();
  {
    std::vector<YOut> yo(yjobs.size());
    const int nthr = (int)std::max<size_t>(1, std::min<size_t>({yjobs.size() / 8 + 1, pcap,
                                                                (size_t)std::max(1u, std::thread::hardware_concurrency())}));
    std::atomic<size_t> next{0};
    auto work = [&]() {
      for (size_t e = next.fetch_add(1); e < yjobs.size(); e = next.fetch_add(1))
        pack_y(P, sweep_lanes_greedy, yjobs[e], yo[e]);
    };
    run_pool(nthr, work);
    const double ty1 = tnow();
    const size_t ny = yo.size();
#define SK_YBIG(X) X(ysc) X(ycs) X(ye2) X(yn_a) X(yn_b) X(yn_c) X(yn_p0) X(yrec) X(yn_w) X(yn_nbp) X(yn_P)
#define SK_OFF(f) std::vector<size_t> off_##f(ny + 1, 0);
    SK_YBIG(SK_OFF)
#undef SK_OFF
    for (size_t e = 0; e < ny; ++e) {
      YOut& Y = yo[e];
      if (!Y.err.empty()) {
        err = Y.err;
        return SK_ERR_INVALID;
      }
#define SK_ACC(f) off_##f[e + 1] = off_##f[e] + Y.f.size();
      SK_YBIG(SK_ACC)
#undef SK_ACC
      P.ex_ysc_base.push_back((int32_t)(off_ysc[e] / 64));
      P.ex_ycs_base.push_back((int32_t)off_ycs[e]);
      P.ex_nch.push_back(Y.nch);
      P.max_nch = std::max(P.max_nch, Y.nch);
    }
#define SK_SIZE(f) P.f.resize(off_##f[ny]);
    SK_YBIG(SK_SIZE)
#undef SK_SIZE
    next = 0;
    auto copy = [&]() {
      for (size_t e = next.fetch_add(1); e < ny; e = next.fetch_add(1)) {
        YOut& Y = yo[e];
#define SK_CPY(f) std::copy(Y.f.begin(), Y.f.end(), P.f.begin() + off_##f[e]);
        SK_YBIG(SK_CPY)
#undef SK_CPY
        Y = YOut();
      }
    };
    run_pool(nthr, copy);
#undef SK_YBIG
    if (tstats) {
      long tch = 0;
      for (int32_t c : P.ex_nch) tch += c;
      fprintf(stderr, "[sk pack] y-role %.1f ms (%d threads) + append %.1f ms; sweep chunks %ld (%.2f per y)\n",
              ty1 - tp2, nthr, tnow() - ty1, tch, P.ex_nch.empty() ? 0.0 : (double)tch / P.ex_nch.size());
    }
  }
  return SK_OK;
}

}

extern "C" {

int sk_dataset_upload(sk_context* ctx, sk_dataset* ds) {
  if (!ctx || !ds) return SK_ERR_INVALID;
  if (ds->uploaded) return ds->device == ctx->device ? SK_OK : sk::fail(ctx, SK_ERR_INVALID, "dataset bound to another device");
  SK_HIP(ctx, hipSetDevice(ctx->device));
  if (sk::ds_pal(ds)) {
    size_t m = 0;
    for (const sk::Example& X : ds->ex) m += X.pal_key.size();
    if (m > (size_t)INT32_MAX) return sk::fail(ctx, SK_ERR_UNSUPPORTED, "palindrome dataset too large");
    try {
      sk::pack_palindromes(ds);
    } catch (const std::bad_alloc&) {
      return sk::fail(ctx, SK_ERR_ALLOC, "palindrome pack");
    }
    const sk_dataset::PalPack& Q = ds->spack;
    SK_HIP(ctx, sk::upload(ds->buf, Q.ex_off, &ds->sdev.ex_off));
    SK_HIP(ctx, sk::upload(ds->buf, Q.key, &ds->sdev.key));
    SK_HIP(ctx, sk::upload(ds->buf, Q.dist, &ds->sdev.dist));
    SK_HIP(ctx, sk::upload(ds->buf, Q.w, &ds->sdev.w));
    ds->spack.key = std::vector<uint64_t>();
    ds->spack.dist = std::vector<int32_t>();
    ds->spack.w = std::vector<float>();
    ds->device = ctx->device;
    ds->uploaded = true;
    return SK_OK;
  }
  if (sk::ds_protein(ds)) {
    size_t pos = 0;
    for (const sk::Example& X : ds->ex) pos += (size_t)X.len;
    if (pos > (size_t)INT32_MAX) return sk::fail(ctx, SK_ERR_UNSUPPORTED, "protein dataset too large");
    try {
      sk::pack_protein(ds);
    } catch (const std::bad_alloc&) {
      return sk::fail(ctx, SK_ERR_ALLOC, "protein pack");
    }
    const sk_dataset::ProtPack& Q = ds->ppack;
    SK_HIP(ctx, sk::upload(ds->buf, Q.ex_len, &ds->pdev.ex_len));
    SK_HIP(ctx, sk::upload(ds->buf, Q.ex_pos_base, &ds->pdev.ex_pos_base));
    SK_HIP(ctx, sk::upload(ds->buf, Q.prof, &ds->pdev.prof));
    SK_HIP(ctx, sk::upload(ds->buf, Q.code, &ds->pdev.code));
    ds->ppack.prof = std::vector<float>();
    ds->ppack.code = std::vector<uint8_t>();
    ds->device = ctx->device;
    ds->uploaded = true;
    return SK_OK;
  }
  std::string err;
  sk::HostPack& P = ds->pack;
  sk::DevSet& D = ds->dev;
  sk::DeviceBuffers& B = ds->buf;
  const bool stats = std::getenv("SK_HOST_STATS") != nullptr;
  const auto tu0 = std::chrono::steady_clock::now();
  std::thread xt;
  hipError_t xe = hipSuccess;
  double x_ms = 0.0;
  auto up_x = [&]() -> hipError_t {
    hipError_t e = hipSetDevice(ctx->device);
    if (e != hipSuccess) return e;
#define SK_UPX(f, d) \
  if ((e = sk::upload(B, P.f, &D.d)) != hipSuccess) return e;
    SK_UPX(ex_nl, ex_nl)
    SK_UPX(ex_node_base, ex_node_base)
    SK_UPX(ex_edge_base, ex_edge_base)
    SK_UPX(ex_bpf_base, ex_bpf_base)
    SK_UPX(ex_lvl_base, ex_lvl_base)
    SK_UPX(ex_nlev, ex_nlev)
    SK_UPX(ex_nseqs, ex_nseqs)
    SK_UPX(ex_len, ex_len)
    SK_UPX(ex_pos_base, ex_pos_base)
    SK_UPX(ex_has_w, ex_has_w)
    SK_UPX(nd_a, nd_a)
    SK_UPX(nd_b, nd_b)
    SK_UPX(nd_c, nd_c)
    SK_UPX(nd_w, nd_w)
    SK_UPX(nd_nbp, nd_nbp)
    SK_UPX(nd_P, nd_P)
    SK_UPX(ed, ed)
    SK_UPX(bpf_code, bpf_code)
    SK_UPX(bpf_p, bpf_p)
    SK_UPX(lvl, lvl)
    SK_UPX(pos_prof, pos_prof)
    SK_UPX(pos_w, pos_w)
    SK_UPX(pos_chr, pos_chr)
    SK_UPX(pos_lru, pos_lru)
    SK_UPX(ex_nslots, ex_nslots)
    SK_UPX(ex_xch_base, ex_xch_base)
    SK_UPX(xrow, xrow)
    SK_UPX(xr_node, xr_node)
    SK_UPX(xr_ch, xr_ch)
    SK_UPX(xgrow, xgrow)
    SK_UPX(xg_node, xg_node)
    SK_UPX(xg_ch, xg_ch)
    SK_UPX(xg_clg, xg_clg)
    SK_UPX(xg_cpf, xg_cpf)
    SK_UPX(ex_xg_base, ex_xg_base)
    SK_UPX(ex_nlxg, ex_nlxg)
    SK_UPX(ex_xgch_base, ex_xgch_base)
    SK_UPX(gr_info, gr_info)
    SK_UPX(gr_pf, gr_pf)
    SK_UPX(gr_P, gr_P)
    SK_UPX(ex_gapless, ex_gapless)
    SK_UPX(gam_key, gam_key)
    SK_UPX(xg_cty, xg_cty)
    SK_UPX(gra_gidx, gra_gidx)
    SK_UPX(gra_row, gra_row)
    SK_UPX(phk_idx, phk_idx)
    SK_UPX(phi_al, phi_al)
    SK_UPX(phi_g, phi_g)
    {
      std::vector<int32_t> grb = P.ex_gr_base;
      grb.push_back((int32_t)P.gr_info.size());
      if ((e = sk::upload(B, grb, &D.ex_gr_base)) != hipSuccess) return e;
      std::vector<int32_t> b1 = P.ex_gra_base, b2 = P.ex_phk_base;
      b1.push_back((int32_t)P.gra_gidx.size());
      b2.push_back((int32_t)P.phk_idx.size());
      if ((e = sk::upload(B, b1, &D.ex_gra_base)) != hipSuccess) return e;
      if ((e = sk::upload(B, b2, &D.ex_phk_base)) != hipSuccess) return e;
    }
#undef SK_UPX
    return hipSuccess;
  };
  const std::function<void()> after_x = [&]() {
    P.xr_ch.insert(P.xr_ch.end(), 8, 0u);
    P.xg_ch.insert(P.xg_ch.end(), 8, 0u);
    auto job = [&]() {
      const auto t0 = std::chrono::steady_clock::now();
      xe = up_x();
      x_ms = std::chrono::duration<double, std::milli>(std::chrono::steady_clock::now() - t0).count();
    };
    try {
      xt = std::thread(job);
    } catch (const std::system_error&) {
      job();
    }
  };
  int rc = sk::pack_dataset(ds, err, &after_x);
  if (xt.joinable()) xt.join();
  if (rc) return sk::fail(ctx, rc, err);
  SK_HIP(ctx, xe);
  const auto tu1 = std::chrono::steady_clock::now();
  D.n_examples = (int32_t)ds->ex.size();
  SK_HIP(ctx, sk::upload(B, P.yn_a, &D.yn_a));
  SK_HIP(ctx, sk::upload(B, P.yn_b, &D.yn_b));
  SK_HIP(ctx, sk::upload(B, P.yn_w, &D.yn_w));
  SK_HIP(ctx, sk::upload(B, P.yn_nbp, &D.yn_nbp));
  SK_HIP(ctx, sk::upload(B, P.yn_P, &D.yn_P));
  SK_HIP(ctx, sk::upload(B, P.ysc, &D.ysc));
  SK_HIP(ctx, sk::upload(B, P.ye2, &D.ye2));
  SK_HIP(ctx, sk::upload(B, P.yn_c, &D.yn_c));
  SK_HIP(ctx, sk::upload(B, P.yn_p0, &D.yn_p0));
  SK_HIP(ctx, sk::upload(B, P.ycs, &D.ycs));
  SK_HIP(ctx, sk::upload(B, P.yrec, &D.yrec));
  SK_HIP(ctx, sk::upload(B, P.ex_ysc_base, &D.ex_ysc_base));
  SK_HIP(ctx, sk::upload(B, P.ex_nch, &D.ex_nch));
  SK_HIP(ctx, sk::upload(B, P.ex_ycs_base, &D.ex_ycs_base));
  D.n_gam = (int32_t)P.gam_key.size();
  D.n_phi = (int32_t)P.phi_al.size();
  D.max_nl = P.max_nl;
  D.max_edges = P.max_edges;
  D.max_bpf = P.max_bpf;
  D.max_nlev = P.max_nlev;
  D.max_nch = P.max_nch;
  D.max_len = P.max_len;
  D.max_slots = P.max_slots;
  D.total_nodes = (int64_t)P.nd_a.size();
  ds->device = ctx->device;
  ds->uploaded = true;
  if (stats) {
    const auto tu2 = std::chrono::steady_clock::now();
    std::fprintf(stderr,
                 "[sk upload] pack + x-role arrays %.1f ms (x-role transfer %.1f ms beside the y-role pack), %zu arrays "
                 "%.1f MB in all, y-role transfer %.1f ms\n",
                 std::chrono::duration<double, std::milli>(tu1 - tu0).count(), x_ms, B.ptrs.size(), B.bytes / 1e6,
                 std::chrono::duration<double, std::milli>(tu2 - tu1).count());
  }
  return SK_OK;
}

int sk_dataset_pack_digest(sk_dataset* ds, uint64_t* y_hash, uint64_t* x_hash) {
  if (!ds || !y_hash || !x_hash) return SK_ERR_INVALID;
  if (ds->uploaded) return SK_ERR_INVALID;
  auto hv = [](const auto& v, uint64_t h) {
    typedef typename std::decay_t<decltype(v)>::value_type T;
    const unsigned char* p = reinterpret_cast<const unsigned char*>(v.data());
    for (size_t i = 0; i < v.size() * sizeof(T); ++i) h = (h ^ p[i]) * 1099511628211ull;
    return h ^ v.size();
  };
  uint64_t hy = 1469598103934665603ull, hx = hy;
  if (sk::ds_pal(ds)) {
    try {
      sk::pack_palindromes(ds);
    } catch (const std::bad_alloc&) {
      return SK_ERR_ALLOC;
    }
    const sk_dataset::PalPack& Q = ds->spack;
    *y_hash = hv(Q.w, hv(Q.dist, hv(Q.key, hy)));
    *x_hash = hv(Q.ex_off, hx);
    ds->spack = sk_dataset::PalPack();
    return SK_OK;
  }
  if (sk::ds_protein(ds)) {
    try {
      sk::pack_protein(ds);
    } catch (const std::bad_alloc&) {
      return SK_ERR_ALLOC;
    }
    const sk_dataset::ProtPack& Q = ds->ppack;
    *y_hash = hv(Q.code, hv(Q.prof, hy));
    *x_hash = hv(Q.ex_coded, hv(Q.ex_pos_base, hv(Q.ex_len, hx)));
    ds->ppack = sk_dataset::ProtPack();
    return SK_OK;
  }
  std::string err;
  const int rc = sk::pack_dataset(ds, err);
  if (rc) return rc;
  const sk::HostPack& P = ds->pack;
#define SK_DG_Y(f) hy = hv(P.f, hy);
#define SK_DG_X(f) hx = hv(P.f, hx);
  SK_PACK_Y_ARRAYS(SK_DG_Y)
  SK_PACK_X_ARRAYS(SK_DG_X)
#undef SK_DG_Y
#undef SK_DG_X
  *y_hash = hy;
  *x_hash = hx;
  ds->pack = sk::HostPack();
  return SK_OK;
}

}
```

stem_kernel_amd/csrc/host/pairs_dag.cpp:

```cpp
#include <hip/hip_runtime.h>

#include <algorithm>
#include <atomic>
#include <chrono>
#include <cmath>
#include <cstdio>
#include <cstdlib>
#include <string>
#include <vector>

#include "host/runtime_types.h"
#include "ribosum85_60.inc"

namespace sk {
namespace {

struct StemClass {
  int maxk = 0;
  int max_nl = 0, max_edges = 0, max_bpf = 0, max_nch = 0;
  int nwaves = 1, grid = 1;
  size_t item_off = 0, n_items = 0;
  size_t slot_off = 0, n_slots = 0;
  bool gam_shared = false;
  bool phi_shared = false;
// ... 226 lines not shown
}

int run_dag_pairs(sk_context* ctx, sk_dataset* xs_, sk_dataset* ys_, const sk_kernel_params* kp,
                      const int32_t* x, const int32_t* y, int64_t n, double* out_dev) {
  int rc = SK_OK;
  const int ny = (int)ys_->ex.size();
  const bool stem = kind_has_stem(kp->kind), str = kind_has_str(kp->kind);
  const HostPack& PX = xs_->pack;
  const HostPack& PY = ys_->pack;
  const bool host_stats = std::getenv("SK_HOST_STATS") != nullptr;
  auto now_ms = [] {
    return std::chrono::duration<double, std::milli>(std::chrono::steady_clock::now().time_since_epoch()).count();
  };
  const double th0 = host_stats ? now_ms() : 0.0;
  double th1 = th0, th2 = th0;

  StemPlan plan;
  const int max_len = std::max(PX.max_len, PY.max_len);
  if (stem) {
    rc = plan_stem_items(ctx, PX, PY, x, y, n, ny, max_len, plan);
    if (rc) return rc;
    ctx->last_cells = plan.cells;
  }

  if (host_stats) th1 = now_ms();
  std::vector<int32_t> item_phi_off, item_phi;
  const bool phi_on = stem && !PX.phi_al.empty() && !PX.gam_key.empty();
  bool two_streams = false;
  double *scratch_cls = nullptr, *scratch_tab = nullptr;
  int64_t big_stride = 0, big_wave = 0;
  int big_grid = 0;
  if (stem) {
    two_streams = plan.classes.size() > 1 && !SK_KNOB("SK_SERIAL_CLASSES");
    size_t scratch_need = 0, scratch_x = 0;
    size_t tab_total = 0;
    size_t phi_budget = SIZE_MAX;
    if (const char* e = SK_KNOB("SK_PHI_TABLE_MB")) phi_budget = (size_t)std::max(0.0, std::atof(e) * 1048576.0);
    auto size_classes = [&](size_t gam_budget) {
      scratch_need = scratch_x = tab_total = 0;
      auto gam_bytes = [&](const StemClass& C) {
        return C.n_slots * (size_t)PX.gam_key.size() * (size_t)(64 * C.maxk + 1) * sizeof(double);
      };
      auto phi_bytes = [&](const StemClass& C) {
        return phi_on ? C.n_slots * (size_t)PX.phi_al.size() * (size_t)(64 * C.maxk + 1) * sizeof(double) : 0;
      };
      size_t total = 0, phi_total = 0;
      for (StemClass& C : plan.classes) {
        C.gam_shared = C.n_slots > 0 && total + gam_bytes(C) <= gam_budget;
        if (C.gam_shared) total += gam_bytes(C);
      }
      for (StemClass& C : plan.classes) {
        C.phi_shared = phi_on && C.gam_shared && total + phi_bytes(C) <= gam_budget &&
                       phi_total + phi_bytes(C) <= phi_budget;
        if (C.phi_shared) {
          total += phi_bytes(C);
          phi_total += phi_bytes(C);
        }
      }
      for (size_t c = 0; c < plan.classes.size(); ++c) {
        StemClass& C = plan.classes[c];
        if (C.gam_shared) {
          C.tab_off = tab_total / sizeof(double);
          tab_total += gam_bytes(C) + (C.phi_shared ? phi_bytes(C) : 0);
        }
        const int64_t slab = (int64_t)(PX.max_slots + 1) * 64 * C.maxk;
        const int64_t gtab1 = (int64_t)PX.gam_key.size() * 64 * C.maxk;
        const int64_t ptab = phi_on ? (int64_t)PX.phi_al.size() * (64 * C.maxk + 1) : 0;
        const size_t b = (size_t)C.grid *
                         (C.nwaves * slab + (C.phi_shared ? 0 : ptab) + (C.gam_shared ? 0 : gtab1)) * sizeof(double);
        size_t& r = (two_streams && (c & 1)) ? scratch_x : scratch_need;
        r = std::max(r, b);
      }
    };
    const bool any_slots = !PX.gam_key.empty() && !plan.slot_y.empty();
    size_classes(any_slots ? SIZE_MAX : 0);
    if (const char* e = SK_KNOB("SK_GAM_TABLE_MB")) {
      size_classes((size_t)std::max(0.0, std::atof(e) * 1048576.0));
    } else if (tab_total > 0 && scratch_need + scratch_x + tab_total + 512 > ctx->scratch_bytes) {
      size_t free_b = 0, total_b = 0;
      SK_HIP(ctx, hipMemGetInfo(&free_b, &total_b));
      size_classes(std::min<size_t>((free_b + ctx->scratch_bytes) / 4, (size_t)8 << 30));
    }
    big_stride = ((int64_t)std::max(plan.big_max_nl, 1) + 63) / 64 * 64;
    big_wave = (int64_t)(PX.max_slots + 2) * big_stride;
    if (!plan.big_x.empty()) {
      size_t free_b = 0, total_b = 0;
      SK_HIP(ctx, hipMemGetInfo(&free_b, &total_b));
      const size_t budget = std::max<size_t>(std::min<size_t>(free_b / 2, (size_t)32 << 30),
                                             (size_t)big_wave * 8 * sk::kStemBigWaves);
      const int64_t by_mem = (int64_t)(budget / ((size_t)big_wave * 8 * sk::kStemBigWaves));
      const int64_t by_pairs = ((int64_t)plan.big_x.size() + sk::kStemBigWaves - 1) / sk::kStemBigWaves;
      big_grid = (int)std::max<int64_t>(1, std::min<int64_t>({by_mem, by_pairs, (int64_t)ctx->n_cu * 8}));
      scratch_need = std::max(scratch_need,
                              (size_t)big_grid * sk::kStemBigWaves * (size_t)big_wave * sizeof(double));
    }
    const size_t big_need = scratch_need;
    auto get_scratch = [&]() {
      scratch_need = (std::max(scratch_need, big_need) + 255) / 256 * 256;
      scratch_x = (scratch_x + 255) / 256 * 256;
      return ensure_scratch(ctx, std::max<size_t>(scratch_need + scratch_x + tab_total, 64));
    };
    rc = get_scratch();
    if (rc && tab_total > 0) {
      (void)hipGetLastError();
      size_classes(0);
      rc = get_scratch();
    }
    if (rc) return rc;
    scratch_cls = ctx->scratch + scratch_need / sizeof(double);
    scratch_tab = scratch_cls + scratch_x / sizeof(double);
  }
  bool phi_items = false;
  for (const StemClass& C : plan.classes) phi_items = phi_items || (phi_on && !C.phi_shared);
  if (phi_items) {
    const size_t W = (PX.phi_al.size() + 63) / 64;
    const size_t ni = plan.items.size();
    std::vector<uint8_t> own(ni, 0);
    for (const StemClass& C : plan.classes)
      if (!C.phi_shared) std::fill(own.begin() + C.item_off, own.begin() + C.item_off + C.n_items, 1);
    const int T = plan_threads((int)(ni / 512 + 1));
    std::vector<std::vector<int32_t>> tkeys(T), tcnt(T);
    run_slices(T, [&](int t) {
      std::vector<uint64_t> acc(W);
      for (size_t i = ni * t / T; i < ni * (t + 1) / T; ++i) {
        const int4 it = plan.items[i];
        const size_t k0 = tkeys[t].size();
        if (own[i] && PY.ex_gapless[it.x]) {
          std::fill(acc.begin(), acc.end(), 0ull);
          for (int u = it.y; u < it.y + it.z; ++u) {
            const uint64_t* b = PX.ex_phi_bits.data() + (size_t)plan.ixs[u] * W;
            for (size_t w = 0; w < W; ++w) acc[w] |= b[w];
          }
          for (size_t w = 0; w < W; ++w)
            for (uint64_t m = acc[w]; m; m &= m - 1) tkeys[t].push_back((int32_t)(w * 64 + __builtin_ctzll(m)));
        }
        tcnt[t].push_back((int32_t)(tkeys[t].size() - k0));
      }
    });
    item_phi_off.assign(1, 0);
    for (int t = 0; t < T; ++t) {
      item_phi.insert(item_phi.end(), tkeys[t].begin(), tkeys[t].end());
      for (int32_t c : tcnt[t]) item_phi_off.push_back(item_phi_off.back() + c);
    }
  }
  if (phi_on && std::getenv("SK_PHI_STATS")) {
    size_t shared = 0, slots = 0;
    for (const StemClass& C : plan.classes) {
      shared += C.phi_shared ? 1 : 0;
      slots += C.phi_shared ? C.n_slots : 0;
    }
    std::fprintf(stderr, "[phi] keys=%zu items=%zu item keys=%zu pairs=%lld phi components=%zu rows=%zu "
                 "classes=%zu sharing=%zu tables=%zu\n",
                 PX.phi_al.size(), plan.items.size(), item_phi.size(), (long long)n, PX.phk_idx.size(),
                 PX.xgrow.size(), plan.classes.size(), shared, slots);
  }

  if (host_stats) th2 = now_ms();
  const StrPlan splan = order_str_pairs(PX, PY, kp, str, x, y, n);
  const size_t n_str_pos = splan.n_sfast ? PX.pos_prof.size() + (ys_ == xs_ ? 0 : PY.pos_prof.size()) : 0;

  const size_t nb = (size_t)n;
  size_t need = 0;
  need += splan.soidx.size() * 8 + n_str_pos * (2 * sizeof(sk::StrPos) + sizeof(sk::StrCode)) + 1024;
  need += (item_phi_off.size() + item_phi.size()) * 4 + 512;
  need += 256 * 8 + 16 * 8 + (size_t)(max_len + 4) * 8 * 2;
  need += 1024 + 256;
  need += plan.items.size() * sizeof(int4) + nb * (4 + 8) + nb * 8 * 2 + nb * 4 * 2 + 64 + 8 * 256;
  need += plan.slot_y.size() * 4 + 256;
  need += plan.big_x.size() * (4 + 4 + 8) + 3 * 256;
  need += 16 * 256;
  rc = ensure_work(ctx, need);
  if (rc) return rc;
  Arena A{static_cast<char*>(ctx->work), 0, ctx->work_bytes};
  double* d_co = A.take<double>(256);
  double* d_gp_loop = A.take<double>(max_len + 4);
  double* d_st = A.take<double>(16);
  double* d_gp_str = A.take<double>(max_len + 4);
  int4* d_items = A.take<int4>(std::max<size_t>(plan.items.size(), 1));
  int32_t* d_ixs = A.take<int32_t>(std::max<size_t>(nb, 1));
  int64_t* d_oidx = A.take<int64_t>(std::max<size_t>(nb, 1));
  double* d_stem = A.take<double>(nb);
  double* d_str = A.take<double>(nb);
  int32_t* d_px = A.take<int32_t>(nb);
  int32_t* d_py = A.take<int32_t>(nb);
  int* d_ctr = A.take<int>(128);
  int32_t* d_sloty = A.take<int32_t>(std::max<size_t>(plan.slot_y.size(), 1));
  int32_t* d_bx = A.take<int32_t>(std::max<size_t>(plan.big_x.size(), 1));
  int32_t* d_by = A.take<int32_t>(std::max<size_t>(plan.big_x.size(), 1));
  int64_t* d_bo = A.take<int64_t>(std::max<size_t>(plan.big_x.size(), 1));
  int32_t* d_iphi_off = A.take<int32_t>(std::max<size_t>(item_phi_off.size(), 1));
  int32_t* d_iphi = A.take<int32_t>(std::max<size_t>(item_phi.size(), 1));
  int64_t* d_soidx = splan.soidx.empty() ? nullptr : A.take<int64_t>(splan.soidx.size());
  sk::StrPos* d_stab = (splan.n_sfast > splan.n_soh) ? A.take<sk::StrPos>(2 * n_str_pos) : nullptr;
  sk::StrCode* d_ctab = splan.n_soh ? A.take<sk::StrCode>(n_str_pos) : nullptr;

  std::vector<double> co(256), st(16);
  const bool subst = kind_subst(kp->kind);
  for (int k = 0; k < 256; ++k)
    co[k] = subst ? std::exp(SK_RIBOSUM_P[k] * kp->beta)
                  : ((k >> 4) == (k & 15) ? kp->stack : kp->covar);
  for (int k = 0; k < 16; ++k)
    st[k] = subst ? std::exp(SK_RIBOSUM_S[k] * kp->alpha)
                  : ((k >> 2) == (k & 3) ? kp->match : kp->mismatch);
  const std::vector<double> gl = gap_powers(kp->loop_gap, max_len + 4);
  const std::vector<double> gs = gap_powers(kp->gap, max_len + 4);
  hipStream_t S = ctx->stream;
  SK_HIP(ctx, sk::h2d(ctx, d_co, co.data(), 256 * 8, S));
  SK_HIP(ctx, sk::h2d(ctx, d_st, st.data(), 16 * 8, S));
  SK_HIP(ctx, sk::h2d(ctx, d_gp_loop, gl.data(), gl.size() * 8, S));
  SK_HIP(ctx, sk::h2d(ctx, d_gp_str, gs.data(), gs.size() * 8, S));
  SK_HIP(ctx, hipMemsetAsync(d_ctr, 0, 128 * sizeof(int), S));

  double* stem_out = (combine_mode(kp->kind) == sk::kCombineStem) ? out_dev : d_stem;
  double* str_out = (combine_mode(kp->kind) == sk::kCombineStr) ? out_dev : d_str;

  const bool side = stem && str;
  if (str) {
    SK_HIP(ctx, sk::h2d(ctx, d_px, splan.spx.empty() ? x : splan.spx.data(), nb * 4, S));
    SK_HIP(ctx, sk::h2d(ctx, d_py, splan.spy.empty() ? y : splan.spy.data(), nb * 4, S));
    if (d_soidx)
      SK_HIP(ctx, sk::h2d(ctx, d_soidx, splan.soidx.data(), splan.soidx.size() * 8, S));
    if (side) {
      SK_HIP(ctx, hipEventRecord(ctx->evf, S));
      SK_HIP(ctx, hipStreamWaitEvent(ctx->side, ctx->evf, 0));
    }
  }
  if (stem) {
    SK_HIP(ctx, sk::h2d(ctx, d_items, plan.items.data(), plan.items.size() * sizeof(int4), S));
    SK_HIP(ctx, sk::h2d(ctx, d_ixs, plan.ixs.data(), nb * 4, S));
    SK_HIP(ctx, sk::h2d(ctx, d_oidx, plan.ioidx.data(), nb * 8, S));
    SK_HIP(ctx, sk::h2d(ctx, d_sloty, plan.slot_y.data(), plan.slot_y.size() * 4, S));
    if (phi_items) {
      SK_HIP(ctx, sk::h2d(ctx, d_iphi_off, item_phi_off.data(), item_phi_off.size() * 4, S));
      if (!item_phi.empty())
        SK_HIP(ctx, sk::h2d(ctx, d_iphi, item_phi.data(), item_phi.size() * 4, S));
    }
    const double gap2 = kp->loop_gap * kp->loop_gap;
    const size_t nnd = std::max<size_t>(PX.nd_a.size(), 1);
    const size_t nxc = std::max<size_t>(PX.xr_ch.size(), 1), nxg = std::max<size_t>(PX.xgrow.size(), 1),
                 nxgc = std::max<size_t>(PX.xg_ch.size(), 1),
                 ngh = std::max<size_t>(PX.ex_nl.size() * PX.gam_key.size(), 1),
                 nphk = std::max<size_t>(PX.phk_idx.size(), 1);
    if (!xs_->prep) {
      void* p = nullptr;
      SK_HIP(ctx, hipMalloc(&p, (3 * nnd + nxc + nxg + nxgc + ngh + nphk) * sizeof(double)));
      xs_->prep = static_cast<double*>(p);
      xs_->buf.ptrs.push_back(p);
      xs_->prep_loop_gap = -1.0;
    }
    sk::DevParamNodes pn;
    pn.nd_L = xs_->prep;
    pn.nd_SL = xs_->prep + nnd;
    pn.xr_SL = xs_->prep + 2 * nnd;
    pn.xr_chw = xs_->prep + 3 * nnd;
    pn.xg_SL = pn.xr_chw + nxc;
    pn.xg_chw = pn.xg_SL + nxg;
    pn.gam_h = pn.xg_chw + nxgc;
    pn.phk_w = pn.gam_h + ngh;
    if (!(xs_->prep_loop_gap == kp->loop_gap)) {
      SK_HIP(ctx, sk::launch_prep(xs_->dev, pn, d_gp_loop, gap2, S));
      xs_->prep_loop_gap = kp->loop_gap;
    }
#ifdef SK_STAMPS
    unsigned long long* d_stamps = nullptr;
    SK_HIP(ctx, hipMalloc(&d_stamps, 16 * sizeof(unsigned long long)));
    SK_HIP(ctx, hipMemsetAsync(d_stamps, 0, 16 * sizeof(unsigned long long), S));
#endif
    if (host_stats)
      std::fprintf(stderr, "[host] pairs=%lld plan %.2f ms, phi keys %.2f ms, uploads+prep %.2f ms\n",
                   (long long)n, th1 - th0, th2 - th1, now_ms() - th2);
    SK_HIP(ctx, hipEventRecord(ctx->ev0, S));
    std::vector<sk::StemLaunch> launches(plan.classes.size());
    for (size_t c = 0; c < plan.classes.size(); ++c) {
      const StemClass& C = plan.classes[c];
      const bool on_cls = two_streams && (c & 1);
      sk::StemLaunch& SL = launches[c];
      SL.xset = xs_->dev;
      SL.yset = ys_->dev;
      SL.pn = pn;
      SL.co_subst = d_co;
      SL.gpow = d_gp_loop;
      SL.n_gpow = max_len + 2;
      SL.n_gpow_pad = (SL.n_gpow + 1) & ~1;
      SL.gap2 = gap2;
      SL.band = kp->len_band;
      SL.lds_max_nl = 64 * C.maxk;
      SL.lds_max_edges = (C.max_edges + 3) & ~3;
      SL.lds_max_bpf = (C.max_bpf + 1 + 3) & ~3;
      SL.lds_max_nch = C.max_nch + 2;
      SL.lds_max_len_pad = (max_len + 2 + 3) & ~3;
      SL.items = d_items + C.item_off;
      SL.n_items = (int32_t)C.n_items;
      SL.xs = d_ixs;
      SL.oidx = d_oidx;
      SL.out = stem_out;
      SL.item_counter = d_ctr + 16 + sk::kStemQueues * (int)c;
      for (int q = 0; q <= sk::kStemQueues; ++q) SL.queue_off[q] = C.queue_off[q];
      SL.slab_doubles = (int64_t)(PX.max_slots + 1) * SL.lds_max_nl;
      SL.scratch = on_cls ? scratch_cls : ctx->scratch;
      SL.gam_on = !PX.gam_key.empty();
      SL.gam_doubles = (int64_t)PX.gam_key.size() * SL.lds_max_nl;
      double* wg_tab = SL.scratch + (size_t)C.grid * C.nwaves * SL.slab_doubles;
      SL.gam_shared = C.gam_shared ? 1 : 0;
      SL.n_slots = C.gam_shared ? (int32_t)C.n_slots : 0;
      SL.slot_y = d_sloty + C.slot_off;
      SL.gam = C.gam_shared ? scratch_tab + C.tab_off : wg_tab;
      SL.kap_y = SL.gam + C.n_slots * (size_t)SL.gam_doubles;
      SL.phi_on = phi_on ? 1 : 0;
      SL.phi_shared = C.phi_shared ? 1 : 0;
      SL.phi_doubles = phi_on ? (int64_t)PX.phi_al.size() * (SL.lds_max_nl + 1) : 0;
      SL.phi = C.phi_shared ? SL.kap_y + C.n_slots * PX.gam_key.size()
                            : wg_tab + (C.gam_shared ? 0 : (size_t)C.grid * SL.gam_doubles);
      SL.item_phi_off = d_iphi_off + (phi_items ? C.item_off : 0);
      SL.item_phi = d_iphi;
#ifdef SK_STAMPS
      SL.stamps = d_stamps;
#endif
    }
    bool any_tables = false;
    for (size_t c = 0; c < plan.classes.size(); ++c) {
      SK_HIP(ctx, sk::launch_gamma_tables(launches[c], plan.classes[c].nwaves, S));
      any_tables = any_tables || plan.classes[c].gam_shared;
    }
    if (two_streams || (side && any_tables)) SK_HIP(ctx, hipEventRecord(ctx->evk, S));
    if (two_streams) SK_HIP(ctx, hipStreamWaitEvent(ctx->cls, ctx->evk, 0));
    if (side && any_tables) SK_HIP(ctx, hipStreamWaitEvent(ctx->side, ctx->evk, 0));
    for (size_t c = 0; c < plan.classes.size(); ++c) {
      const StemClass& C = plan.classes[c];
      const bool on_cls = two_streams && (c & 1);
      const sk::StemLaunch& SL = launches[c];
      SK_HIP(ctx, sk::lev_mark(ctx, on_cls ? ctx->cls : S));
      SK_HIP(ctx, sk::launch_stem(SL, C.grid, C.nwaves, on_cls ? ctx->cls : S));
      SK_HIP(ctx, sk::lev_mark(ctx, on_cls ? ctx->cls : S));
      if (C.gam_shared && (C.phi_shared || !phi_on)) ++ctx->last_gamma_shared;
      ctx->last_stem_classes |= 1u << (C.maxk % 4 ? C.maxk : C.maxk / 4);
    }
    if (two_streams) {
      SK_HIP(ctx, hipEventRecord(ctx->evx, ctx->cls));
      SK_HIP(ctx, hipStreamWaitEvent(S, ctx->evx, 0));
    }
    if (!plan.big_x.empty()) {
      const size_t nbig = plan.big_x.size();
      SK_HIP(ctx, sk::h2d(ctx, d_bx, plan.big_x.data(), nbig * 4, S));
      SK_HIP(ctx, sk::h2d(ctx, d_by, plan.big_y.data(), nbig * 4, S));
      SK_HIP(ctx, sk::h2d(ctx, d_bo, plan.big_o.data(), nbig * 8, S));
      sk::StemBigLaunch BL;
      BL.xset = xs_->dev;
      BL.yset = ys_->dev;
      BL.pn = pn;
      BL.co_subst = d_co;
      BL.gpow = d_gp_loop;
      BL.n_gpow = max_len + 2;
      BL.gap2 = gap2;
      BL.band = kp->len_band;
      BL.xs = d_bx;
      BL.ys = d_by;
      BL.oidx = d_bo;
      BL.n_pairs = (int64_t)nbig;
      BL.out = stem_out;
      BL.scratch = ctx->scratch;
      BL.stride = big_stride;
      BL.wave_doubles = big_wave;
      SK_HIP(ctx, sk::lev_mark(ctx, S));
      SK_HIP(ctx, sk::launch_stem_big(BL, big_grid, S));
      SK_HIP(ctx, sk::lev_mark(ctx, S));
      ctx->last_stem_classes |= 1u;
    }
    SK_HIP(ctx, hipEventRecord(ctx->ev1, S));
#ifdef SK_STAMPS
    {
      unsigned long long h[16];
      SK_HIP(ctx, hipMemcpyAsync(h, d_stamps, sizeof(h), hipMemcpyDeviceToHost, S));
      SK_HIP(ctx, hipStreamSynchronize(S));
      (void)hipFree(d_stamps);
      const double rows = (double)h[8];
      std::fprintf(stderr, "[stamps] classes=%zu pairs=%llu rows=%.0f cycles/row:", plan.classes.size(),
                   h[9], rows);
      const char* nm[7] = {"hdr", "A", "Rfill", "passes", "zero", "sweep", "store"};
      for (int i = 0; i < 7; ++i) std::fprintf(stderr, " %s=%.0f", nm[i], h[i] / rows);
      std::fprintf(stderr, "\n[stamps] per row: A-loaded rows=%.3f swept chunks=%.2f match passes=%.2f band nodes=%.1f\n",
                   h[10] / rows, h[11] / rows, h[12] / rows, h[13] / rows);
      for (const StemClass& C : plan.classes)
        std::fprintf(stderr, "[stamps] class maxk=%d max_nl=%d max_edges=%d max_nch=%d waves/wg=%d grid=%d items=%zu\n",
                     C.maxk, C.max_nl, C.max_edges, C.max_nch, C.nwaves, C.grid, C.n_items);
    }
#endif
    ctx->last_launches = (int32_t)plan.classes.size() + (plan.big_x.empty() ? 0 : 1);
  }
  if (str) {
    const hipStream_t SS = side ? ctx->side : S;
    sk::StrLaunch T;
    T.xset = xs_->dev;
    T.yset = ys_->dev;
// ... 78 lines not shown
```

stem_kernel_amd/csrc/host/runtime_types.h:

```cpp
#pragma once

#include <hip/hip_runtime.h>

#include <algorithm>
#include <cstdint>
#include <cstring>
#include <functional>
#include <memory>
#include <mutex>
#include <new>
#include <string>
#include <system_error>
#include <thread>
#include <utility>
#include <vector>

#include "stem_kernel.h"
#include "host/runtime.h"
#include "host/sk_internal.h"
#include "kernels/device_set.h"
#include "kernels/launch.h"

namespace sk {

struct DeviceBuffers {
  std::vector<void*> ptrs;
  size_t bytes = 0;
  ~DeviceBuffers() { release(); }
  void release() {
    for (void* p : ptrs) (void)hipFree(p);
    ptrs.clear();
  }
};

template <class V, class T = typename V::value_type>
hipError_t upload(DeviceBuffers& db, const V& v, const T** out) {
  void* p = nullptr;
  const size_t bytes = std::max<size_t>(v.size() * sizeof(T), 16);
  hipError_t e = hipMalloc(&p, bytes);
  if (e != hipSuccess) return e;
  db.ptrs.push_back(p);
  db.bytes += bytes;
  if (!v.empty()) e = hipMemcpy(p, v.data(), v.size() * sizeof(T), hipMemcpyHostToDevice);
  *out = static_cast<const T*>(p);
  return e;
}

template <class T>
struct NoInitAlloc : std::allocator<T> {
  template <class U>
  struct rebind {
    using other = NoInitAlloc<U>;
  };
  NoInitAlloc() = default;
  template <class U>
  NoInitAlloc(const NoInitAlloc<U>&) noexcept {}
  template <class U>
  void construct(U* p) noexcept {
    ::new ((void*)p) U;
  }
  template <class U, class... A>
  void construct(U* p, A&&... a) {
    ::new ((void*)p) U(std::forward<A>(a)...);
  }
};
template <class T>
using pvec = std::vector<T, NoInitAlloc<T>>;

struct HostPack {
  std::vector<int32_t> ex_nl, ex_node_base, ex_edge_base, ex_bpf_base, ex_lvl_base, ex_nlev,
      ex_len, ex_pos_base, ex_has_w;
  std::vector<uint8_t> ex_dyadic;
  std::vector<uint8_t> ex_str_fast, ex_onehot;
  std::vector<uint8_t> ex_big;
  std::vector<float> ex_nseqs;
  pvec<uint32_t> nd_a, nd_b, nd_c;
  pvec<float> nd_w, nd_nbp;
  pvec<double> nd_P;
  pvec<uint2> ed;
  pvec<uint32_t> bpf_code;
  pvec<float> bpf_p;
  pvec<int32_t> lvl;
  pvec<float4> pos_prof;
  pvec<float> pos_w;
  pvec<uint8_t> pos_chr;
  pvec<float4> pos_lru;
  std::vector<int32_t> ex_nslots, ex_xch_base;
  pvec<sk::XRow> xrow;
  pvec<uint32_t> yn_a, yn_b, yn_c, ye2, ysc;
  pvec<uint4> yrec;
  pvec<float> yn_w, yn_nbp, yn_p0;
  pvec<double> yn_P;
  pvec<int32_t> ycs;
  std::vector<int32_t> ex_ysc_base, ex_nch, ex_ycs_base;
  pvec<uint32_t> xr_node, xr_ch;
  pvec<sk::XRow> xgrow;
  std::vector<uint32_t> gam_key;
  pvec<uint32_t> xg_node, xg_ch, xg_clg, gr_info;
  pvec<float> xg_cpf, gr_pf;
  pvec<double> gr_P;
  std::vector<int32_t> ex_xg_base, ex_nlxg, ex_xgch_base, ex_gr_base, ex_gapless;
  pvec<uint8_t> xg_cty;
  std::vector<uint32_t> phi_al, phi_g;
  pvec<uint32_t> gra_gidx, gra_row, phk_idx;
  std::vector<int32_t> ex_gra_base, ex_phk_base;
  pvec<uint64_t> ex_phi_bits;
  int32_t max_nl = 0, max_edges = 0, max_bpf = 0, max_nlev = 0, max_len = 0, max_slots = 0;
  int32_t max_nch = 0;
};
#define SK_PACK_Y_ARRAYS(X) X(yn_a) X(yn_b) X(yn_c) X(ye2) X(ysc) X(yrec) X(yn_w) X(yn_nbp) X(yn_p0) X(yn_P) \
  X(ycs) X(ex_ysc_base) X(ex_nch) X(ex_ycs_base)
#define SK_PACK_X_ARRAYS(X) X(nd_a) X(nd_b) X(nd_c) X(nd_w) X(nd_nbp) X(nd_P) X(ed) X(bpf_code) X(bpf_p)     \
  X(lvl) X(xr_ch) X(xrow) X(xr_node) X(gr_info) X(gr_pf) X(gr_P) X(xg_ch) X(xg_clg) X(xg_cpf) X(xg_cty)     \
  X(phk_idx) X(gra_gidx) X(gra_row) X(xgrow) X(xg_node) X(pos_prof) X(pos_w) X(pos_chr) X(pos_lru)          \
  X(ex_phi_bits) X(ex_nl) X(ex_node_base) X(ex_edge_base) X(ex_bpf_base) X(ex_lvl_base) X(ex_nlev) X(ex_len) \
  X(ex_pos_base) X(ex_has_w) X(ex_dyadic) X(ex_str_fast) X(ex_onehot) X(ex_big) X(ex_nseqs) X(ex_nslots)    \
  X(ex_xch_base) X(gam_key) X(ex_xg_base) X(ex_nlxg) X(ex_xgch_base) X(ex_gr_base) X(ex_gapless) X(phi_al)   \
  X(phi_g) X(ex_gra_base) X(ex_phk_base)

struct Stem4dTables {
  Stem4dTables() = default;
  Stem4dTables(const Stem4dTables&) = delete;
  Stem4dTables& operator=(const Stem4dTables&) = delete;
  ~Stem4dTables() {
    if (device < 0 || buf.ptrs.empty()) return;
    int cur = -1;
    if (hipGetDevice(&cur) != hipSuccess) cur = -1;
    if (hipSetDevice(device) == hipSuccess) (void)hipDeviceSynchronize();
    buf.release();
    if (cur >= 0) (void)hipSetDevice(cur);
  }
  DeviceBuffers buf;
  int device = -1, model = -1;
  unsigned loop = 0;
  size_t n_ex = 0;
  const float* bp = nullptr;
  const uint8_t* ch = nullptr;
  std::vector<int64_t> bp_off, ch_off;
  std::vector<uint8_t> why, acgu;
};

}

struct sk_dataset {
  std::vector<sk::Example> ex;
  std::vector<std::string> labels;
  int device = -1;
  bool uploaded = false;
  sk::DevSet dev;
  sk::DeviceBuffers buf;
  sk::HostPack pack;
  struct ProtPack {
    std::vector<int32_t> ex_len, ex_pos_base;
    std::vector<uint8_t> ex_coded, code;
    std::vector<float> prof;
  } ppack;
  sk::LaProtSet pdev;
  struct PalPack {
    std::vector<int32_t> ex_off, dist;
    std::vector<uint64_t> key;
    std::vector<float> w;
  } spack;
  sk::SimpalSet sdev;
  std::string err;
  double* prep = nullptr;
  double prep_loop_gap = -1.0;
  std::mutex s4_mu;
  std::vector<std::shared_ptr<sk::Stem4dTables>> s4;
};

namespace sk {

constexpr size_t kS4Sets = 4;

enum { kSortRna = 0, kSortProtein = 1, kSortPal = 2 };
inline int ex_sort(const Example& X) { return X.pal ? kSortPal : X.protein ? kSortProtein : kSortRna; }
inline bool ds_protein(const sk_dataset* ds) { return !ds->ex.empty() && ds->ex[0].protein; }
inline bool ds_pal(const sk_dataset* ds) { return !ds->ex.empty() && ds->ex[0].pal; }
inline bool ds_mixes(sk_dataset* ds, int sort) {
  if (ds->ex.empty() || ex_sort(ds->ex[0]) == sort) return false;
  static const char* const name[3] = {"RNA", "protein", "palindrome"};
  static const char* const art[3] = {"an", "a", "a"};
  ds->err = std::string(name[sort]) + " example added to " + art[ex_sort(ds->ex[0])] + " " +
            name[ex_sort(ds->ex[0])] + " dataset";
  return true;
}
inline bool pal_seed_differs(sk_dataset* ds, int32_t seed_length) {
  if (!ds_pal(ds) || ds->ex[0].pal_seed == seed_length) return false;
  ds->err = "palindrome example of another seed_length than the dataset's";
  return true;
}
struct Stem4dBatch {
  sk::Stem4dPair* pairs = nullptr;
  int2* items = nullptr;
  int32_t* band = nullptr;
  size_t cap_pairs = 0, cap_items = 0, cap_band = 0;
};

}

struct sk_context {
  sk::Stem4dBatch s4d;
  int device = 0;
  hipStream_t stream = nullptr;
  bool own_stream = false;
  int n_cu = 0;
  std::string err;
  double* scratch = nullptr;
  size_t scratch_bytes = 0;
  void* work = nullptr;
  size_t work_bytes = 0;
  hipEvent_t ev0 = nullptr, ev1 = nullptr, ev2 = nullptr, ev3 = nullptr;
  hipStream_t side = nullptr;
  hipEvent_t evf = nullptr, evj = nullptr;
  hipStream_t cls = nullptr;
  hipEvent_t evk = nullptr, evx = nullptr;
  hipStream_t aux = nullptr;
  hipEvent_t eva = nullptr;
  struct TSet {
    hipEvent_t ev[4] = {nullptr, nullptr, nullptr, nullptr};
    std::vector<hipEvent_t> lev;
    size_t lev_used = 0;
    bool pending = false, stem = false, str = false;
    double cells = 0.0;
    int32_t launches = 0;
  };
  static constexpr int kTSets = 4;
  TSet tset[kTSets];
  int tk = 0;
  bool async = false;
  double acc_stem_ms = 0.0, acc_str_ms = 0.0, acc_cells = 0.0, acc_launch_ms = 0.0;
  int32_t acc_launch_n = 0, acc_launches = 0;
  struct Stage {
    std::vector<std::pair<char*, size_t>> blocks;
    size_t blk = 0, off = 0;
    hipEvent_t ev = nullptr;
    bool recorded = false;
    char* dbuf = nullptr;
    size_t dcap = 0;
    hipEvent_t uev = nullptr;
  };
  Stage stage[2];
  hipStream_t cps = nullptr;
  uint64_t ncalls = 0;
  double last_launch_ms_sum = 0.0;
  int32_t last_launch_n = 0;
  double last_stem_ms = 0.0, last_str_ms = 0.0, last_cells = 0.0;
  int32_t last_launches = 0;
  uint32_t last_stem_classes = 0, last_s4d_classes = 0;
  int32_t last_gamma_shared = 0;
  uint32_t last_la_protein = 0;
  void* comm = nullptr;
};

namespace sk {

template <class F>
void run_slices(int n, F&& f) {
  std::vector<std::thread> th;
  std::vector<int> here;
  for (int t = 1; t < n; ++t) {
    try {
// ... 111 lines not shown
```

stem_kernel_amd/kernel_matrix.py:

```python
from __future__ import annotations

import ctypes as C
import sys
from typing import Iterable, List, Optional, Sequence

import numpy as np

from . import _lib
from ._lib import SK_OK, KernelParams, StemKernelError, check, lib

__all__ = [
    "fold", "random_sequences", "Dataset", "Context", "KernelMatrix",
    "SuStemKernel", "SiStemKernel", "StringKernel", "SuStemStrKernel", "StemStrKernel",
    "SiStemStrKernel", "LSuStemKernel", "LSuStemStrKernel", "NaiveStringKernel",
    "StemKernelError", "SVMModel", "LAKernel", "SimpalKernel", "simpal_shape",
]


_FORMATS = {"fa": _lib.FMT_FASTA, "fasta": _lib.FMT_FASTA, "aln": _lib.FMT_CLUSTAL,
            "clustal": _lib.FMT_CLUSTAL, "maf": _lib.FMT_MAF}


def _seqfile_rows(h) -> List[List[str]]:
    L = lib()
# ... 289 lines not shown
        check(lib().sk_dataset_palindromes(self._h, i, None, kb, d.ctypes.data_as(C.POINTER(C.c_int32)),
                                           w.ctypes.data_as(C.POINTER(C.c_float))))
        raw = kb.raw.rstrip(b"\0")
        s = len(raw) // m if m else 0
        return [raw[k * s:(k + 1) * s].decode() for k in range(m)], d[:m], w[:m]

    def add_file(self, label: str, path: str, fmt: str = "fa", th: float = 0.01,
                 use_bp: bool = True, protein: bool = False) -> int:
        alns = read_examples(path, fmt)
        for rows in alns:
            if protein:
                self.add_protein(label, rows)
            else:
                self.add(label, rows, th=th, use_bp=use_bp)
        return len(alns)

    @classmethod
    def from_sequences(cls, seqs: Iterable[str], labels: Optional[Iterable[str]] = None,
                       th: float = 0.01, bpp: Optional[Sequence[np.ndarray]] = None):
        ds = cls()
        seqs = list(seqs)
        labels = list(labels) if labels is not None else ["+1"] * len(seqs)
        for k, s in enumerate(seqs):
            ds.add(labels[k], [s], None if bpp is None else [bpp[k]], th=th)
        return ds

    @classmethod
    def synthetic(cls, seqs: Sequence[str], labels: Optional[Sequence[str]] = None,
                  th: float = 0.01, threads: int = 0):
        ds = cls()
        n = len(seqs)
        sarr = (C.c_char_p * n)(*[s.encode() for s in seqs])
        larr = None if labels is None else (C.c_char_p * n)(*[l.encode() for l in labels])
        check(lib().sk_dataset_add_synthetic(ds._h, n, sarr, larr, C.c_float(th), threads))
        return ds

    @classmethod
    def synthetic_alignments(cls, alns: Sequence[Sequence[str]], labels=None, th: float = 0.01,
                             threads: int = 0):
        ds = cls()
        n = len(alns)
        nr = len(alns[0]) if n else 1
        if any(len(a) != nr for a in alns):
            raise ValueError("synthetic_alignments needs the same number of rows per alignment")
        flat = [r.encode() for a in alns for r in a]
        rarr = (C.c_char_p * max(len(flat), 1))(*flat)
        larr = None if labels is None else (C.c_char_p * n)(*[l.encode() for l in labels])
        check(lib().sk_dataset_add_synthetic_rows(ds._h, n, nr, rarr, larr, C.c_float(th),
                                                  threads))
        return ds

    def add_batch(self, alns: Sequence[Sequence[str]], bpp_rows=None, labels=None,
                  th: float = 0.01, use_bp: bool = True, threads: int = 0) -> None:
        n = len(alns)
        nr = len(alns[0]) if n else 1
        if any(len(a) != nr for a in alns):
            raise ValueError("add_batch needs the same number of rows per alignment")
        flat = [r.encode() for a in alns for r in a]
        rarr = (C.c_char_p * max(len(flat), 1))(*flat)
        larr = None if labels is None else (C.c_char_p * n)(*[l.encode() for l in labels])
        keep, barr = [], None
        if use_bp:
            barr = (C.POINTER(C.c_double) * max(n * nr, 1))()
            for i in range(n):
                for r in range(nr):
                    b = np.ascontiguousarray(bpp_rows[i][r], dtype=np.float64)
                    if b.size == 0:
                        b = np.zeros(1)
                    keep.append(b)
                    barr[i * nr + r] = b.ctypes.data_as(C.POINTER(C.c_double))
        check(lib().sk_dataset_add_batch(self._h, n, nr, rarr, barr, larr, C.c_float(th),
                                         int(use_bp), threads))

    @classmethod
    def folded(cls, ctx: "Context", alns, labels=None, th: float = 0.01, no_gu: bool = False,
               no_closing_gu: bool = False, threads: int = 0, no_lonely_pairs: bool = False,
               n_samples: int = 0, seed: int = 0, consensus: bool = False):
        alns = [[a] if isinstance(a, str) else list(a) for a in alns]
        ds = cls()
        n = len(alns)
        nr = len(alns[0]) if n else 1
        if any(len(a) != nr for a in alns):
            raise ValueError("folded needs the same number of rows per alignment")
        flat = [r.encode() for a in alns for r in a]
        rarr = (C.c_char_p * max(len(flat), 1))(*flat)
        larr = None if labels is None else (C.c_char_p * n)(*[l.encode() for l in labels])
        flags = (1 if no_gu else 0) | (2 if no_closing_gu else 0) | (4 if no_lonely_pairs else 0)
        if n_samples < 0:
            raise ValueError("n_samples must not be negative")
        if n_samples > 0:
            ctx._chk(lib().sk_dataset_add_sampled(ctx.handle, ds._h, n, nr, rarr, larr, C.c_float(th),
                                                  flags, n_samples, seed, threads))
        elif consensus:
            ctx._chk(lib().sk_dataset_add_alifolded(ctx.handle, ds._h, n, nr, rarr, larr, C.c_float(th),
                                                    flags, threads))
        else:
            ctx._chk(lib().sk_dataset_add_folded(ctx.handle, ds._h, n, nr, rarr, larr, C.c_float(th),
                                                 flags, threads))
        return ds

    def __len__(self):
        return lib().sk_dataset_size(self._h)

    def export(self, first: int = 0, count: Optional[int] = None) -> bytearray:
        count = len(self) - first if count is None else count
        need = C.c_size_t()
        check(lib().sk_dataset_export(self._h, first, count, None, 0, C.byref(need)))
        out = bytearray(need.value)
        buf = (C.c_char * max(need.value, 1)).from_buffer(out) if need.value else None
        check(lib().sk_dataset_export(self._h, first, count, buf, need.value, C.byref(need)))
        return out

    def import_bytes(self, data) -> "Dataset":
        n = len(data)
        if isinstance(data, bytearray) and n:
            data = (C.c_char * n).from_buffer(data)
        check(lib().sk_dataset_import(self._h, data, n))
        return self

    def pack_digest(self):
        hy, hx = C.c_uint64(), C.c_uint64()
        check(lib().sk_dataset_pack_digest(self._h, C.byref(hy), C.byref(hx)))
        return hy.value, hx.value

    def profile(self, i: int):
        L = self.shape(i)[4]
        out = np.zeros((max(L, 1), 5), np.float32)
        ns = C.c_float()
        check(lib().sk_dataset_profile(self._h, i, out.ctypes.data_as(C.POINTER(C.c_float)),
                                       C.byref(ns)))
        return out[:L], ns.value

    def bpla_weights(self, i: int):
        L = self.shape(i)[4]
        a = [np.zeros(max(L, 1), np.float32) for _ in range(3)]
        check(lib().sk_dataset_bpla_weights(self._h, i, *(v.ctypes.data_as(C.POINTER(C.c_float))
                                                           for v in a)))
        return [v[:L] for v in a]

    def label(self, i: int) -> str:
        return lib().sk_dataset_label(self._h, i).decode()

    def shape(self, i: int):
        v = [C.c_int32() for _ in range(5)]
        check(lib().sk_dataset_shape(self._h, i, *[C.byref(a) for a in v]))
        return tuple(a.value for a in v)

    def row_traffic(self, i: int) -> dict:
        v = [C.c_int32() for _ in range(7)]
        check(lib().sk_dataset_row_traffic(self._h, i, *[C.byref(a) for a in v]))
        return dict(zip(("rows", "stored", "slab_reads", "gamma_reads", "phi_reads", "reg_reads",
                         "y_slots"), (a.value for a in v)))

    def dag(self, i: int) -> dict:
        nn, ne, nb, nr, L = self.shape(i)
        u = lambda k: np.zeros(max(k, 1), np.uint32)
        f = lambda k: np.zeros(max(k, 1), np.float32)
        d = dict(first=u(nn), last=u(nn), n_edges=u(nn), n_bpfreq=u(nn), weight=f(nn),
                 max_pa=u(nn), edge_to=u(ne), edge_gaps=u(ne), bp_code=u(nb), bp_p=f(nb),
                 roots=u(nr), pos_weight=f(L))
        ptr = lambda a: a.ctypes.data_as(C.POINTER(C.c_uint32 if a.dtype == np.uint32 else C.c_float))
        check(lib().sk_dataset_dag(self._h, i, *[ptr(d[k]) for k in
                                                 ("first", "last", "n_edges", "n_bpfreq", "weight",
                                                  "max_pa", "edge_to", "edge_gaps", "bp_code",
                                                  "bp_p", "roots", "pos_weight")]))
        sizes = dict(first=nn, last=nn, n_edges=nn, n_bpfreq=nn, weight=nn, max_pa=nn,
                     edge_to=ne, edge_gaps=ne, bp_code=nb, bp_p=nb, roots=nr, pos_weight=L)
        return {k: v[: sizes[k]] for k, v in d.items()}


class Context:

    def __init__(self, device: int = 0, stream: Optional[int] = None):
        self._h = C.c_void_p()
        check(lib().sk_open(device, C.c_void_p(stream) if stream else None, C.byref(self._h)))
        self.device = device

    def close(self):
        if self._h is not None and self._h.value:
            lib().sk_close(self._h)
            self._h = None

    def __del__(self):
        try:
            self.close()
        except Exception:
            pass

    @property
    def handle(self):
        return self._h

    def _chk(self, rc):
        return check(rc, self._h)

    def fold(self, seqs: Sequence[str], no_gu: bool = False, no_closing_gu: bool = False,
             log_z: bool = False, no_lonely_pairs: bool = False):
        seqs = list(seqs)
        n = len(seqs)
        sizes = [len(s) * (len(s) - 1) // 2 for s in seqs]
        out = np.zeros(max(sum(sizes), 1))
        lz = np.zeros(max(n, 1))
        sarr = (C.c_char_p * max(n, 1))(*[s.encode() for s in seqs])
        flags = (1 if no_gu else 0) | (2 if no_closing_gu else 0) | (4 if no_lonely_pairs else 0)
        self._chk(lib().sk_fold_mccaskill(self._h, n, sarr, flags,
                                          out.ctypes.data_as(C.POINTER(C.c_double)),
                                          lz.ctypes.data_as(C.POINTER(C.c_double))))
        res, o = [], 0
        for z in sizes:
            res.append(out[o:o + z].copy())
            o += z
        return (res, lz[:n]) if log_z else res

    def fold_alignment(self, alns: Sequence[Sequence[str]], no_gu: bool = False,
                       no_lonely_pairs: bool = False, with_log_z: bool = False):
        alns = [[a] if isinstance(a, str) else list(a) for a in alns]
        n = len(alns)
        sizes = [len(a[0]) * (len(a[0]) - 1) // 2 if a else 0 for a in alns]
        out = np.zeros(max(sum(sizes), 1))
        lz = np.zeros(max(n, 1))
        flat = [r.encode() for a in alns for r in a]
        rarr = (C.c_char_p * max(len(flat), 1))(*flat)
        nrow = np.array([len(a) for a in alns] or [0], dtype=np.int32)
        flags = (1 if no_gu else 0) | (4 if no_lonely_pairs else 0)
        self._chk(lib().sk_fold_alignment(self._h, n, nrow.ctypes.data_as(C.POINTER(C.c_int32)), rarr, flags,
                                          out.ctypes.data_as(C.POINTER(C.c_double)),
                                          lz.ctypes.data_as(C.POINTER(C.c_double))))
        res, o = [], 0
        for z in sizes:
            res.append(out[o:o + z].copy())
            o += z
        return (res, lz[:n]) if with_log_z else res

    def fold_sample(self, seqs: Sequence[str], n_samples: int, seed: int = 0, no_gu: bool = False,
                    no_closing_gu: bool = False, no_lonely_pairs: bool = False,
                    structures: bool = False, log_z: bool = False):
        seqs = list(seqs)
        n = len(seqs)
        sizes = [len(s) * (len(s) - 1) // 2 for s in seqs]
        out = np.zeros(max(sum(sizes), 1))
        lz = np.zeros(max(n, 1))
        sarr = (C.c_char_p * max(n, 1))(*[s.encode() for s in seqs])
        flags = (1 if no_gu else 0) | (2 if no_closing_gu else 0) | (4 if no_lonely_pairs else 0)
        sbuf = None
        if structures:
            sbuf = np.zeros(max(sum(len(s) for s in seqs) * max(n_samples, 0), 1), np.uint8)
        self._chk(lib().sk_fold_sample(self._h, n, sarr, flags, n_samples, seed,
                                       out.ctypes.data_as(C.POINTER(C.c_double)),
                                       sbuf.ctypes.data if structures else None,
                                       lz.ctypes.data_as(C.POINTER(C.c_double))))
        res, o = [], 0
        for z in sizes:
            res.append(out[o:o + z].copy())
            o += z
        ret = [res]
        if structures:
            raw, strs, o = sbuf.tobytes(), [], 0
            for s in seqs:
                m = len(s)
                strs.append([raw[o + k * m:o + (k + 1) * m].decode("ascii") for k in range(n_samples)])
                o += m * n_samples
            ret.append(strs)
        if log_z:
            ret.append(lz[:n])
        return ret[0] if len(ret) == 1 else tuple(ret)

    def upload(self, ds: Dataset):
        self._chk(lib().sk_dataset_upload(self._h, ds.handle))

    def gram(self, ds: Dataset, kernel: _Kernel, normalize: bool = False) -> np.ndarray:
        self.upload(ds)
        n = len(ds)
        out = np.zeros((n, n), dtype=np.float64)
        self._chk(lib().sk_gram(self._h, ds.handle, C.byref(kernel.params), int(normalize),
                                out.ctypes.data_as(C.POINTER(C.c_double))))
        return out

    def pairs(self, ds: Dataset, kernel: _Kernel, x, y) -> np.ndarray:
        self.upload(ds)
        x = np.ascontiguousarray(x, dtype=np.int32)
        y = np.ascontiguousarray(y, dtype=np.int32)
        out = np.zeros(x.size, dtype=np.float64)
        self._chk(lib().sk_pairs(self._h, ds.handle, C.byref(kernel.params),
                                 x.ctypes.data_as(C.POINTER(C.c_int32)),
                                 y.ctypes.data_as(C.POINTER(C.c_int32)), x.size,
                                 out.ctypes.data_as(C.POINTER(C.c_double))))
        return out

    def bpla_gradients(self, ds: Dataset, kernel: "BPLAKernel", x, y, ys: Optional[Dataset] = None):
        ys = ds if ys is None else ys
        self.upload(ds)
        self.upload(ys)
        x = np.ascontiguousarray(x, dtype=np.int32)
        y = np.ascontiguousarray(y, dtype=np.int32)
        val = np.zeros(x.size, dtype=np.float64)
        grad = np.zeros((x.size, 4), dtype=np.float64)
        self._chk(lib().sk_bpla_gradients(self._h, ds.handle, ys.handle, C.byref(kernel.params),
                                          x.ctypes.data_as(C.POINTER(C.c_int32)),
                                          y.ctypes.data_as(C.POINTER(C.c_int32)), x.size,
                                          val.ctypes.data_as(C.POINTER(C.c_double)),
                                          grad.ctypes.data_as(C.POINTER(C.c_double))))
        return val, grad

    def bpla_gradient_gram(self, ds: Dataset, kernel: "BPLAKernel", normalize: bool = False):
        from .shard import assemble_gradients
        n = len(ds)
# ... 214 lines not shown
```

Measured before the change: 229,300.

## Factor common child sums across DAG rows into shared intermediate rows

Adds a host-side scheduler that finds groups of children (same gap offsets) appearing in several DAG rows and replaces them with a single shared-sum row, then reorders rows and reassigns storage slots. The device then runs this factored row schedule in place of the original gamma schedule, which should cut the per-pair inner-loop child reads and multiply-adds. The cost is extra pack-time work, extra intermediate rows and slot pressure. The schedule falls back to the original when constraints fail.

```diff
diff --git a/include/stem_kernel.h b/include/stem_kernel.h
--- a/include/stem_kernel.h
+++ b/include/stem_kernel.h
@@ -110,6 +110,8 @@
 int sk_dataset_row_traffic(const sk_dataset *ds, int i, int32_t *rows, int32_t *stored,
                            int32_t *slab_reads, int32_t *gamma_reads, int32_t *phi_reads,
                            int32_t *reg_reads, int32_t *y_slots);
+int sk_dataset_shared_sums(const sk_dataset *ds, int i, int32_t *shared_rows,
+                           int32_t *member_records);
 int sk_dataset_dag(const sk_dataset *ds, int i, uint32_t *first, uint32_t *last,
                    uint32_t *n_edges, uint32_t *n_bpfreq, float *weight,
                    uint32_t *max_pa, uint32_t *edge_to, uint32_t *edge_gaps,
diff --git a/stem_kernel_amd/_lib.py b/stem_kernel_amd/_lib.py
--- a/stem_kernel_amd/_lib.py
+++ b/stem_kernel_amd/_lib.py
@@ -113,6 +113,7 @@
     "sk_dataset_label": (C.c_char_p, [_P, C.c_int]),
     "sk_dataset_shape": (C.c_int, [_P, C.c_int, _I32P, _I32P, _I32P, _I32P, _I32P]),
     "sk_dataset_row_traffic": (C.c_int, [_P, C.c_int, _I32P, _I32P, _I32P, _I32P, _I32P, _I32P, _I32P]),
+    "sk_dataset_shared_sums": (C.c_int, [_P, C.c_int, _I32P, _I32P]),
     "sk_dataset_dag": (C.c_int, [_P, C.c_int, _U32P, _U32P, _U32P, _U32P, _F32P, _U32P,
                                  _U32P, _U32P, _U32P, _F32P, _U32P, _F32P]),
     "sk_dataset_profile": (C.c_int, [_P, C.c_int, _F32P, _F32P]),
diff --git a/stem_kernel_amd/csrc/host/dataset.cpp b/stem_kernel_amd/csrc/host/dataset.cpp
--- a/stem_kernel_amd/csrc/host/dataset.cpp
+++ b/stem_kernel_amd/csrc/host/dataset.cpp
@@ -442,26 +442,39 @@
   if ((int)P.ex_nlxg.size() != (int)ds->ex.size()) return SK_ERR_INVALID;
   int32_t st = 0, sl = 0, ga = 0, ph = 0, rg = 0;
   uint32_t prev = 0xffffu;
-  size_t k = (size_t)P.ex_xgch_base[i];
-  for (size_t r = (size_t)P.ex_xg_base[i]; r < (size_t)P.ex_xg_base[i] + P.ex_nlxg[i]; ++r) {
-    const int ne = P.xgrow[r].a & 0xff;
+  const auto& rows_ = P.run_rows();
+  const auto& ch_ = P.run_ch();
+  const int32_t nlr = P.run_nl()[i];
+  size_t k = (size_t)P.run_ch_base()[i];
+  for (size_t r = (size_t)P.run_base()[i]; r < (size_t)P.run_base()[i] + nlr; ++r) {
+    const int ne = rows_[r].a & 0xff;
     for (int t = 0; t < ne; ++t, ++k) {
-      const uint32_t c = P.xg_ch[k] & 0xffffu;
+      const uint32_t c = ch_[k] & 0xffffu;
       if (c == prev) ++rg;
       else if (c & 0x8000u) ++ga;
       else if (c & 0x4000u) ++ph;
       else ++sl;
     }
-    prev = P.xgrow[r].b >> 16;
+    prev = rows_[r].b >> 16;
     st += prev < 0x4000u;
   }
-  if (rows) *rows = P.ex_nlxg[i];
+  if (rows) *rows = nlr;
   if (stored) *stored = st;
   if (slab_reads) *slab_reads = sl;
   if (gamma_reads) *gamma_reads = ga;
   if (phi_reads) *phi_reads = ph;
   if (reg_reads) *reg_reads = rg;
   if (y_slots) *y_slots = P.ex_nl[i];
+  return SK_OK;
+}
+
+int sk_dataset_shared_sums(const sk_dataset* ds, int i, int32_t* shared_rows, int32_t* member_records) {
+  if (!ds) return SK_ERR_INVALID;
+  if (i < 0 || i >= (int)ds->ex.size()) return SK_ERR_RANGE;
+  const sk::HostPack& P = ds->pack;
+  if ((int)P.ex_nlxg.size() != (int)ds->ex.size()) return SK_ERR_INVALID;
+  if (shared_rows) *shared_rows = P.shared_sums ? P.ex_ss_rows[i] : 0;
+  if (member_records) *member_records = P.shared_sums ? P.ex_ss_repl[i] : 0;
   return SK_OK;
 }
 
diff --git a/stem_kernel_amd/csrc/host/pack.cpp b/stem_kernel_amd/csrc/host/pack.cpp
--- a/stem_kernel_amd/csrc/host/pack.cpp
+++ b/stem_kernel_amd/csrc/host/pack.cpp
@@ -16,6 +16,7 @@
 #include <utility>
 #include <vector>
 
+#include "host/pack_shared_sums.h"
 #include "host/runtime_types.h"
 
 namespace sk {
@@ -180,6 +181,8 @@
   std::vector<uint32_t> gam_key;
   std::vector<uint64_t> phi_raw;
   bool gam_on = false, phi_on = false;
+  bool ss_on = false;
+  int ss_thr = 0;
   uint32_t gamma_idx(uint32_t key) const {
     return (uint32_t)(std::lower_bound(gam_key.begin(), gam_key.end(), key) - gam_key.begin());
   }
@@ -231,6 +234,8 @@
   std::sort(K.phi_raw.begin(), K.phi_raw.end());
   K.phi_raw.erase(std::unique(K.phi_raw.begin(), K.phi_raw.end()), K.phi_raw.end());
   K.phi_on = K.gam_on && !K.phi_raw.empty() && K.phi_raw.size() < 0x4000 && !SK_KNOB("SK_NO_PHI");
+  K.ss_on = K.gam_on && !SK_KNOB("SK_NO_SHARED_SUMS");
+  if (const char* t = SK_KNOB("SK_SHARED_SUMS_THR")) K.ss_thr = std::atoi(t);
   return K;
 }
 
@@ -383,6 +388,11 @@
   std::vector<sk::XRow> xrow, xgrow;
   std::vector<float4> pos_prof, pos_lru;
   std::vector<uint64_t> ex_phi_bits;
+  std::vector<sk::XRow> xf_row;
+  std::vector<uint32_t> xf_node, xf_ch, xf_clg, xf_gra_row;
+  std::vector<float> xf_cpf;
+  std::vector<uint8_t> xf_cty;
+  int ss_rows = 0, ss_repl = 0;
   int nl = 0, nlev = 0, max_slots = 0, n_nostore = 0, n_nodes = 0, gslots = 0;
   bool big = false;
   int rc = SK_OK;
@@ -677,6 +687,11 @@
           if (X.edge_to[k] == v) nostore[v] = 1;
       }
     }
+    std::vector<sk::SsRow> ss_in;
+    std::vector<int32_t> grow_of(nn, -1);
+    std::vector<uint32_t> ss_gra;
+    if (K.ss_on) ss_in.reserve(order.size());
+    uint32_t ss_key = (uint32_t)nn;
     for (int v : order) {
       const uint32_t e0 = X.edge_off[v], e1 = X.edge_off[v + 1];
       const uint32_t b0 = X.bpf_off[v], b1 = X.bpf_off[v + 1];
@@ -689,6 +704,7 @@
       const bool loop = level[v] == 0;
       const bool phi = (fl[v] & 2) != 0;
       uint32_t nch = 0;
+      const size_t rec0 = O.xg_ch.size();
       if (phi) {
         const uint32_t kp = gamma_key(X, v);
         for (uint32_t k = e0; k < e1; ++k) {
@@ -755,9 +771,60 @@
       xr.P = Pw[v];
       xr.c = (O.nd_b[nid[v]] >> 16) | ((b1 > b0 ? (uint32_t)X.bpf_code[b0] : 0u) << 16) |
              (phi ? 0x80000000u : 0u);
+      if (K.ss_on) {
+        sk::SsRow W;
+        W.xr = xr;
+        W.node = (uint32_t)nid[v];
+        W.user = W.swept = !phi && !loop;
+        size_t t = rec0;
+        auto table = [&](uint32_t key) {
+          W.rec.push_back(sk::SsRec{-1, key, O.xg_ch[t] & 0xffffu, O.xg_ch[t] >> 16, O.xg_clg[t], O.xg_cpf[t],
+                                    O.xg_cty[t]});
+          ++t;
+        };
+        if (phi) {
+          for (; t < O.xg_ch.size();) table(ss_key++);
+          ss_gra.push_back((uint32_t)O.xgrow.size());
+        } else if (!loop) {
+          for (uint32_t k = e0; k < e1; ++k) {
+            const int c = X.edge_to[k];
+            if (fl[c] & 1) {
+              table((uint32_t)c);
+            } else {
+              W.rec.push_back(sk::SsRec{grow_of[c], 0u, 0u, X.edge_gaps[k], 0u, 1.0f, 0});
+              ++t;
+            }
+          }
+        }
+        grow_of[v] = (int32_t)O.xgrow.size();
+        ss_in.push_back(std::move(W));
+      }
       O.xgrow.push_back(xr);
       O.xg_node.push_back((uint32_t)nid[v]);
       ++nlxg;
+    }
+    if (K.ss_on) {
+      sk::SsOut F;
+      if (sk::shared_sums_schedule(std::move(ss_in), K.ss_thr, SK_KNOB("SK_STORE_ALL") != nullptr, F)) {
+        O.xf_row.swap(F.row);
+        O.xf_node.swap(F.node);
+        O.xf_ch.swap(F.ch);
+        O.xf_clg.swap(F.clg);
+        O.xf_cpf.swap(F.cpf);
+        O.xf_cty.swap(F.cty);
+        for (uint32_t r : ss_gra) O.xf_gra_row.push_back(F.new_index[r]);
+        O.ss_rows = F.n_shared;
+        O.ss_repl = F.n_replaced;
+        O.max_slots = std::max(O.max_slots, F.nslots);
+      } else {
+        O.xf_row = O.xgrow;
+        O.xf_node = O.xg_node;
+        O.xf_ch = O.xg_ch;
+        O.xf_clg = O.xg_clg;
+        O.xf_cpf = O.xg_cpf;
+        O.xf_cty = O.xg_cty;
+        O.xf_gra_row = O.gra_row;
+      }
     }
     if (K.phi_on) {
       const size_t W = (K.phi_raw.size() + 63) / 64;
@@ -850,6 +917,7 @@
                                                               (size_t)std::max(1u, std::thread::hardware_concurrency())}));
   const KeyTables K = key_tables(ds->ex, nthr);
   P.gam_key = K.gam_key;
+  P.shared_sums = K.ss_on;
   if (K.phi_on)
     for (uint64_t k : K.phi_raw) {
       P.phi_al.push_back((uint32_t)k);
@@ -875,7 +943,7 @@
 #define SK_BIG(X) X(nd_a) X(nd_b) X(nd_c) X(nd_w) X(nd_nbp) X(nd_P) X(ed) X(bpf_code) X(bpf_p) X(lvl) \
   X(xr_ch) X(xrow) X(xr_node) X(gr_info) X(gr_pf) X(gr_P) X(xg_ch) X(xg_clg) X(xg_cpf) X(xg_cty)    \
   X(phk_idx) X(gra_gidx) X(gra_row) X(xgrow) X(xg_node) X(pos_prof) X(pos_w) X(pos_chr) X(pos_lru)  \
-  X(ex_phi_bits)
+  X(ex_phi_bits) X(xf_row) X(xf_node) X(xf_ch) X(xf_clg) X(xf_cpf) X(xf_cty) X(xf_gra_row)
 #define SK_OFF(f) std::vector<size_t> off_##f(n + 1, 0);
     SK_BIG(SK_OFF)
 #undef SK_OFF
@@ -900,6 +968,13 @@
       P.ex_gr_base.push_back((int32_t)off_gr_info[e]);
       P.ex_gra_base.push_back((int32_t)off_gra_gidx[e]);
       P.ex_phk_base.push_back((int32_t)off_phk_idx[e]);
+      if (K.ss_on) {
+        P.ex_xf_base.push_back((int32_t)off_xf_row[e]);
+        P.ex_xfch_base.push_back((int32_t)off_xf_ch[e]);
+        P.ex_nlxf.push_back((int32_t)O.xf_row.size());
+        P.ex_ss_rows.push_back(O.ss_rows);
+        P.ex_ss_repl.push_back(O.ss_repl);
+      }
       app(P.ex_big, O.ex_big); app(P.ex_nslots, O.ex_nslots); app(P.ex_nlxg, O.ex_nlxg);
       app(P.ex_gapless, O.ex_gapless); app(P.ex_nl, O.ex_nl); app(P.ex_nlev, O.ex_nlev);
       app(P.ex_nseqs, O.ex_nseqs); app(P.ex_len, O.ex_len); app(P.ex_has_w, O.ex_has_w);
@@ -927,6 +1002,7 @@
         for (int e = nx.fetch_add(1); e < n; e = nx.fetch_add(1)) {
           XOut& O = xo[e];
           for (uint32_t& r : O.gra_row) r += (uint32_t)off_xgrow[e];
+          for (uint32_t& r : O.xf_gra_row) r += (uint32_t)off_xf_row[e];
 #define SK_CPY(f) std::copy(O.f.begin(), O.f.end(), P.f.begin() + off_##f[e]);
           SK_BIG(SK_CPY)
 #undef SK_CPY
@@ -966,6 +1042,32 @@
               "[sk pack] gamma schedule: %ld nodes, %ld rows, %ld unstored, %ld slots; stored %ld, reads: "
               "slab %ld gamma %ld phi %ld, from registers %ld\n",
               s_nodes, s_rows, s_nost, s_slots, s_st, s_slab, s_gam, s_phi, s_reg);
+      if (P.shared_sums) {
+        long f_rows = 0, f_ss = 0, f_repl = 0, f_st = 0, f_slab = 0, f_gam = 0, f_phi = 0, f_reg = 0;
+        for (int e = 0; e < n; ++e) {
+          f_rows += P.ex_nlxf[e];
+          f_ss += P.ex_ss_rows[e];
+          f_repl += P.ex_ss_repl[e];
+          uint32_t prev = 0xffffu;
+          size_t k = (size_t)P.ex_xfch_base[e];
+          for (size_t r = (size_t)P.ex_xf_base[e]; r < (size_t)P.ex_xf_base[e] + P.ex_nlxf[e]; ++r) {
+            const int ne = P.xf_row[r].a & 0xff;
+            for (int t = 0; t < ne; ++t, ++k) {
+              const uint32_t c = P.xf_ch[k] & 0xffffu;
+              if (c == prev) ++f_reg;
+              else if (c & 0x8000u) ++f_gam;
+              else if (c & 0x4000u) ++f_phi;
+              else ++f_slab;
+            }
+            prev = P.xf_row[r].b >> 16;
+            f_st += prev < 0x4000u;
+          }
+        }
+        fprintf(stderr,
+                "[sk pack] factored schedule: %ld rows, %ld shared sums for %ld records; stored %ld, reads: "
+                "slab %ld gamma %ld phi %ld, from registers %ld\n",
+                f_rows, f_ss, f_repl, f_st, f_slab, f_gam, f_phi, f_reg);
+      }
     }
   }
   if (after_x) (*after_x)();
@@ -1117,22 +1219,35 @@
     SK_UPX(xrow, xrow)
     SK_UPX(xr_node, xr_node)
     SK_UPX(xr_ch, xr_ch)
-    SK_UPX(xgrow, xgrow)
-    SK_UPX(xg_node, xg_node)
-    SK_UPX(xg_ch, xg_ch)
-    SK_UPX(xg_clg, xg_clg)
-    SK_UPX(xg_cpf, xg_cpf)
-    SK_UPX(ex_xg_base, ex_xg_base)
-    SK_UPX(ex_nlxg, ex_nlxg)
-    SK_UPX(ex_xgch_base, ex_xgch_base)
+    if (P.shared_sums) {
+      SK_UPX(xf_row, xgrow)
+      SK_UPX(xf_node, xg_node)
+      SK_UPX(xf_ch, xg_ch)
+      SK_UPX(xf_clg, xg_clg)
+      SK_UPX(xf_cpf, xg_cpf)
+      SK_UPX(xf_cty, xg_cty)
+      SK_UPX(xf_gra_row, gra_row)
+      SK_UPX(ex_xf_base, ex_xg_base)
+      SK_UPX(ex_nlxf, ex_nlxg)
+      SK_UPX(ex_xfch_base, ex_xgch_base)
+    } else {
+      SK_UPX(xgrow, xgrow)
+      SK_UPX(xg_node, xg_node)
+      SK_UPX(xg_ch, xg_ch)
+      SK_UPX(xg_clg, xg_clg)
+      SK_UPX(xg_cpf, xg_cpf)
+      SK_UPX(xg_cty, xg_cty)
+      SK_UPX(gra_row, gra_row)
+      SK_UPX(ex_xg_base, ex_xg_base)
+      SK_UPX(ex_nlxg, ex_nlxg)
+      SK_UPX(ex_xgch_base, ex_xgch_base)
+    }
     SK_UPX(gr_info, gr_info)
     SK_UPX(gr_pf, gr_pf)
     SK_UPX(gr_P, gr_P)
     SK_UPX(ex_gapless, ex_gapless)
     SK_UPX(gam_key, gam_key)
-    SK_UPX(xg_cty, xg_cty)
     SK_UPX(gra_gidx, gra_gidx)
-    SK_UPX(gra_row, gra_row)
     SK_UPX(phk_idx, phk_idx)
     SK_UPX(phi_al, phi_al)
     SK_UPX(phi_g, phi_g)
@@ -1152,6 +1267,7 @@
   const std::function<void()> after_x = [&]() {
     P.xr_ch.insert(P.xr_ch.end(), 8, 0u);
     P.xg_ch.insert(P.xg_ch.end(), 8, 0u);
+    if (P.shared_sums) P.xf_ch.insert(P.xf_ch.end(), 8, 0u);
     auto job = [&]() {
       const auto t0 = std::chrono::steady_clock::now();
       xe = up_x();
diff --git a/stem_kernel_amd/csrc/host/pack_shared_sums.cpp b/stem_kernel_amd/csrc/host/pack_shared_sums.cpp
--- /dev/null
+++ b/stem_kernel_amd/csrc/host/pack_shared_sums.cpp
@@ -0,0 +1,351 @@
+#include "host/pack_shared_sums.h"
+
+#include <algorithm>
+#include <utility>
+
+namespace sk {
+namespace {
+
+constexpr int kPairs = 4, kRounds = 3;
+constexpr uint32_t kNear = 8;
+
+inline int32_t rec_id(const SsRec& r) { return r.row >= 0 ? r.row : -1 - (int32_t)r.key; }
+
+struct Cand {
+  uint32_t off, len;
+  uint64_t hash;
+  uint32_t uoff, ulen;
+  long value;
+};
+
+}
+
+bool shared_sums_schedule(std::vector<SsRow>&& in, int threshold, bool store_all, SsOut& out) {
+  const int n = (int)in.size();
+  std::vector<SsRow> R(std::move(in));
+  out = SsOut();
+  int32_t nkeys = 0;
+  for (const SsRow& W : R)
+    if (W.user)
+      for (const SsRec& r : W.rec)
+        if (r.row < 0) nkeys = std::max(nkeys, (int32_t)r.key + 1);
+
+  typedef std::pair<int32_t, uint32_t> Mem;
+  std::vector<Mem> mem, tmp, mem_prev;
+  std::vector<uint32_t> moff(n + 1), moff_prev, poff, pfill;
+  std::vector<int32_t> par, idpool, upool;
+  std::vector<uint32_t> relpool;
+  std::vector<Cand> cands;
+  std::vector<uint32_t> keep;
+  std::vector<int> cnt(n, 0), seen, us;
+  std::vector<std::pair<int64_t, uint32_t>> com;
+  std::vector<uint8_t> touched(n);
+  for (int round = 0; round < kRounds; ++round) {
+    mem.swap(mem_prev);
+    moff.swap(moff_prev);
+    moff.resize(n + 1);
+    mem.clear();
+    for (int u = 0; u < n; ++u) {
+      moff[u] = (uint32_t)mem.size();
+      if (!R[u].user) continue;
+      if (round > 0 && !touched[u]) {
+        mem.insert(mem.end(), mem_prev.begin() + moff_prev[u], mem_prev.begin() + moff_prev[u + 1]);
+        continue;
+      }
+      tmp.clear();
+      for (const SsRec& r : R[u].rec)
+        if (r.cty <= 1) tmp.push_back({rec_id(r), r.gaps});
+      std::sort(tmp.begin(), tmp.end());
+      for (size_t i = 0; i < tmp.size();) {
+        size_t j = i + 1;
+        while (j < tmp.size() && tmp[j].first == tmp[i].first) ++j;
+        if (j == i + 1) mem.push_back(tmp[i]);
+        i = j;
+      }
+    }
+    moff[n] = (uint32_t)mem.size();
+    const int32_t nrow = (int32_t)R.size();
+    auto slot_of = [&](int32_t id) { return id >= 0 ? id : nrow + (-1 - id); };
+    poff.assign((size_t)nrow + nkeys + 1, 0u);
+    for (const Mem& m : mem) ++poff[slot_of(m.first) + 1];
+    for (size_t i = 0; i + 1 < poff.size(); ++i) poff[i + 1] += poff[i];
+    pfill.assign(poff.begin(), poff.end() - 1);
+    par.resize(mem.size());
+    for (int u = 0; u < n; ++u)
+      for (uint32_t i = moff[u]; i < moff[u + 1]; ++i) par[pfill[slot_of(mem[i].first)]++] = u;
+    pfill.assign(poff.begin(), poff.end() - 1);
+    cands.clear();
+    idpool.clear();
+    relpool.clear();
+    for (int u = 0; u < n; ++u) {
+      const Mem* mu = mem.data() + moff[u];
+      const uint32_t nu = moff[u + 1] - moff[u];
+      if (nu < 2) continue;
+      seen.clear();
+      for (uint32_t i = 0; i < nu; ++i) {
+        const int32_t sl = slot_of(mu[i].first);
+        uint32_t& cur = pfill[sl];
+        while (cur < poff[sl + 1] && par[cur] <= u) ++cur;
+        for (uint32_t t = cur; t < poff[sl + 1] && t < cur + kNear; ++t)
+          if (cnt[par[t]]++ == 0) seen.push_back(par[t]);
+      }
+      std::sort(seen.begin(), seen.end());
+      int npair = 0;
+      for (int v : seen) {
+        const int c = cnt[v];
+        cnt[v] = 0;
+        if (c < 2 || npair >= kPairs) continue;
+        if (round > 0 && !touched[u] && !touched[v]) continue;
+        ++npair;
+        const Mem* mv = mem.data() + moff[v];
+        const uint32_t nv = moff[v + 1] - moff[v];
+        com.clear();
+        for (uint32_t i = 0, j = 0; i < nu && j < nv;) {
+          if (mu[i].first < mv[j].first) ++i;
+          else if (mv[j].first < mu[i].first) ++j;
+          else {
+            com.push_back({(int64_t)mu[i].second - (int64_t)mv[j].second, i});
+            ++i, ++j;
+          }
+        }
+        std::sort(com.begin(), com.end());
+        size_t b0 = 0, bl = 0;
+        for (size_t i = 0; i < com.size();) {
+          size_t j = i + 1;
+          while (j < com.size() && com[j].first == com[i].first) ++j;
+          if (j - i > bl) bl = j - i, b0 = i;
+          i = j;
+        }
+        if (bl < 2) continue;
+        Cand cd{(uint32_t)idpool.size(), (uint32_t)bl, 1469598103934665603ull, 0u, 0u, 0};
+        uint32_t mn = 0xffffffffu;
+        for (size_t i = b0; i < b0 + bl; ++i) mn = std::min(mn, mu[com[i].second].second);
+        for (size_t i = b0; i < b0 + bl; ++i) {
+          idpool.push_back(mu[com[i].second].first);
+          relpool.push_back(mu[com[i].second].second - mn);
+          cd.hash = (cd.hash ^ (uint32_t)idpool.back()) * 1099511628211ull;
+        }
+        cands.push_back(cd);
+      }
+    }
+    keep.resize(cands.size());
+    for (size_t i = 0; i < cands.size(); ++i) keep[i] = (uint32_t)i;
+    auto same = [&](const Cand& a, const Cand& b) {
+      return a.hash == b.hash && a.len == b.len &&
+             std::equal(idpool.begin() + a.off, idpool.begin() + a.off + a.len, idpool.begin() + b.off);
+    };
+    std::sort(keep.begin(), keep.end(), [&](uint32_t a, uint32_t b) {
+      return cands[a].hash != cands[b].hash ? cands[a].hash < cands[b].hash : a < b;
+    });
+    {
+      size_t o = 0;
+      for (size_t i = 0; i < keep.size(); ++i) {
+        bool dup = false;
+        for (size_t j = o; j-- > 0 && cands[keep[j]].hash == cands[keep[i]].hash && !dup;)
+          dup = same(cands[keep[j]], cands[keep[i]]);
+        if (!dup) keep[o++] = keep[i];
+      }
+      keep.resize(o);
+    }
+    std::sort(keep.begin(), keep.end());
+    upool.clear();
+    {
+      size_t o = 0;
+      for (uint32_t ci : keep) {
+        Cand& cd = cands[ci];
+        const int32_t* ids = idpool.data() + cd.off;
+        const uint32_t* rel = relpool.data() + cd.off;
+        int32_t least = slot_of(ids[0]);
+        for (uint32_t t = 1; t < cd.len; ++t) {
+          const int32_t sl = slot_of(ids[t]);
+          if (poff[sl + 1] - poff[sl] < poff[least + 1] - poff[least]) least = sl;
+        }
+        cd.uoff = (uint32_t)upool.size();
+        for (uint32_t q = poff[least]; q < poff[least + 1]; ++q) {
+          const int u = par[q];
+          const Mem* mu = mem.data() + moff[u];
+          const uint32_t nu = moff[u + 1] - moff[u];
+          uint32_t i = 0;
+          int64_t d = 0;
+          bool ok = true;
+          for (uint32_t t = 0; t < cd.len && ok; ++t) {
+            while (i < nu && mu[i].first < ids[t]) ++i;
+            ok = i < nu && mu[i].first == ids[t] && mu[i].second >= rel[t];
+            if (!ok) break;
+            const int64_t dt = (int64_t)mu[i].second - rel[t];
+            if (t == 0) d = dt;
+            ok = dt == d;
+          }
+          if (ok) upool.push_back(u);
+        }
+        cd.ulen = (uint32_t)upool.size() - cd.uoff;
+        const long k = (long)cd.ulen, s = (long)cd.len;
+        cd.value = k * s - (s + 1 + k) - threshold;
+        if (k >= 2 && cd.value > 0) keep[o++] = ci;
+      }
+      keep.resize(o);
+    }
+    std::stable_sort(keep.begin(), keep.end(), [&](uint32_t a, uint32_t b) { return cands[a].value > cands[b].value; });
+    std::fill(touched.begin(), touched.end(), 0);
+    int applied = 0;
+    for (uint32_t ci : keep) {
+      const Cand& cd = cands[ci];
+      const int32_t* ids = idpool.data() + cd.off;
+      us.clear();
+      for (uint32_t q = 0; q < cd.ulen; ++q)
+        if (!touched[upool[cd.uoff + q]]) us.push_back(upool[cd.uoff + q]);
+      const long k = (long)us.size(), s = (long)cd.len;
+      if (k < 2 || k * s - (s + 1 + k) - threshold <= 0) continue;
+      const int z = (int)R.size();
+      SsRow Z;
+      Z.xr = XRow{0u, 0u, 0x80000000u, 0.0f, 0.0f, 0.0f, 0.0};
+      Z.node = R[us[0]].node;
+      Z.user = false;
+      Z.swept = false;
+      for (uint32_t t = 0; t < cd.len; ++t)
+        for (const SsRec& r : R[us[0]].rec)
+          if (r.cty <= 1 && rec_id(r) == ids[t]) {
+            SsRec m = r;
+            m.gaps = relpool[cd.off + t];
+            Z.rec.push_back(m);
+          }
+      for (int u : us) {
+        std::vector<SsRec> nr;
+        nr.reserve(R[u].rec.size());
+        uint32_t mg = 0xffffffffu;
+        size_t at = R[u].rec.size();
+        for (const SsRec& r : R[u].rec) {
+          if (r.cty <= 1 && std::binary_search(ids, ids + cd.len, rec_id(r))) {
+            mg = std::min(mg, r.gaps);
+            at = std::min(at, nr.size());
+          } else {
+            nr.push_back(r);
+          }
+        }
+        const SsRec zr{z, 0u, 0u, mg, 0u, 1.0f, 0};
+        nr.insert(nr.begin() + std::min<size_t>(at, 3), zr);
+        R[u].rec.swap(nr);
+        touched[u] = 1;
+        out.n_replaced += (int)s;
+      }
+      R.push_back(std::move(Z));
+      ++out.n_shared;
+      ++applied;
+    }
+    if (!applied) break;
+  }
+
+  const int nr = (int)R.size();
+  std::vector<int> gap(nr, -1);
+  std::vector<int> ready(nr, -1);
+  for (int r = 0; r < n; ++r) ready[r] = r;
+  for (int z = n; z < nr; ++z)
+    for (const SsRec& m : R[z].rec)
+      if (m.row >= 0) ready[z] = std::max(ready[z], ready[m.row]);
+  {
+    std::vector<int> need(nr, n);
+    for (int r = 0; r < n; ++r)
+      for (const SsRec& m : R[r].rec)
+        if (m.row >= n) need[m.row] = std::min(need[m.row], r - 1);
+    for (int z = nr - 1; z >= n; --z) {
+      gap[z] = ready[z] >= 0 ? ready[z] : need[z];
+      for (const SsRec& m : R[z].rec)
+        if (m.row >= n) need[m.row] = std::min(need[m.row], gap[z]);
+    }
+  }
+  std::vector<int> order;
+  order.reserve(nr);
+  {
+    std::vector<int> goff(n + 2, 0), gl(nr - n);
+    for (int z = n; z < nr; ++z) ++goff[gap[z] + 2];
+    for (int i = 0; i <= n; ++i) goff[i + 1] += goff[i];
+    std::vector<int> gf(goff.begin(), goff.end() - 1);
+    for (int z = n; z < nr; ++z) gl[gf[gap[z] + 1]++] = z;
+    for (int g = -1; g < n; ++g) {
+      if (g >= 0) order.push_back(g);
+      for (int i = goff[g + 1]; i < goff[g + 2]; ++i) order.push_back(gl[i]);
+    }
+  }
+  std::vector<int> pos(nr, -1);
+  for (int i = 0; i < nr; ++i) pos[order[i]] = i;
+  for (int i = 1; i < nr; ++i) {
+    const int z = order[i];
+    if (z < n) continue;
+    std::vector<SsRec>& rec = R[z].rec;
+    for (size_t t = 0; t < rec.size(); ++t)
+      if (rec[t].row == order[i - 1]) {
+        std::rotate(rec.begin(), rec.begin() + t, rec.begin() + t + 1);
+        break;
+      }
+  }
+  for (int r = 0; r < nr; ++r) {
+    if (R[r].rec.size() > 255) return false;
+    for (const SsRec& m : R[r].rec)
+      if (m.row >= 0 && pos[m.row] >= pos[r]) return false;
+  }
+
+  std::vector<int> npar(nr, 0), last(nr, -1);
+  for (int i = 0; i < nr; ++i)
+    for (const SsRec& m : R[order[i]].rec)
+      if (m.row >= 0) {
+        ++npar[m.row];
+        last[m.row] = order[i];
+      }
+  std::vector<uint8_t> nostore(nr, 0);
+  for (int i = 0; i + 1 < nr && !store_all; ++i) {
+    const int v = order[i], r = order[i + 1];
+    if (npar[v] != 1 || !(R[r].swept || r >= n)) continue;
+    for (size_t t = 0; t < R[r].rec.size() && t < 4; ++t)
+      if (R[r].rec[t].row == v) nostore[v] = 1;
+  }
+  std::vector<uint32_t> slot(nr, 0xffffu);
+  std::vector<int> freel;
+  int nslots = 0;
+  out.new_index.assign(n, 0u);
+  out.row.reserve(nr);
+  out.node.reserve(nr);
+  {
+    size_t nrec = 0;
+    for (const SsRow& W : R) nrec += W.rec.size();
+    out.ch.reserve(nrec);
+    out.clg.reserve(nrec);
+    out.cpf.reserve(nrec);
+    out.cty.reserve(nrec);
+  }
+  for (int i = 0; i < nr; ++i) {
+    const int v = order[i];
+    const SsRow& W = R[v];
+    for (const SsRec& m : W.rec) {
+      out.ch.push_back((m.row >= 0 ? (slot[m.row] & 0xffffu) : m.lo) | (m.gaps << 16));
+      out.clg.push_back(m.clg);
+      out.cpf.push_back(m.cpf);
+      out.cty.push_back(m.cty);
+      if (m.gaps > 0xffffu) return false;
+    }
+    for (const SsRec& m : W.rec)
+      if (m.row >= 0 && last[m.row] == v && slot[m.row] < 0x4000u) {
+        freel.push_back((int)slot[m.row]);
+        slot[m.row] |= 0x10000u;
+      }
+    if (nostore[v]) {
+      slot[v] = 0xfffeu;
+    } else if (npar[v] > 0) {
+      if (!freel.empty()) {
+        slot[v] = (uint32_t)freel.back();
+        freel.pop_back();
+      } else {
+        slot[v] = (uint32_t)nslots++;
+      }
+    }
+    XRow xr = W.xr;
+    xr.a = (xr.a & ~0xffu) | (uint32_t)W.rec.size();
+    xr.b = (xr.b & 0xffffu) | (slot[v] << 16);
+    out.row.push_back(xr);
+    out.node.push_back(W.node);
+    if (v < n) out.new_index[v] = (uint32_t)i;
+  }
+  out.nslots = nslots;
+  return nslots < 0x4000;
+}
+
+}
diff --git a/stem_kernel_amd/csrc/host/pack_shared_sums.h b/stem_kernel_amd/csrc/host/pack_shared_sums.h
--- /dev/null
+++ b/stem_kernel_amd/csrc/host/pack_shared_sums.h
@@ -0,0 +1,37 @@
+#pragma once
+#include <hip/hip_runtime.h>
+
+#include <cstdint>
+#include <vector>
+
+#include "kernels/device_set.h"
+
+namespace sk {
+
+struct SsRec {
+  int32_t row;
+  uint32_t key;
+  uint32_t lo;
+  uint32_t gaps, clg;
+  float cpf;
+  uint8_t cty;
+};
+struct SsRow {
+  XRow xr;
+  uint32_t node;
+  bool user;
+  bool swept;
+  std::vector<SsRec> rec;
+};
+struct SsOut {
+  std::vector<XRow> row;
+  std::vector<uint32_t> node, ch, clg;
+  std::vector<float> cpf;
+  std::vector<uint8_t> cty;
+  std::vector<uint32_t> new_index;
+  int nslots = 0, n_shared = 0, n_replaced = 0;
+};
+
+bool shared_sums_schedule(std::vector<SsRow>&& in, int threshold, bool store_all, SsOut& out);
+
+}
diff --git a/stem_kernel_amd/csrc/host/pairs_dag.cpp b/stem_kernel_amd/csrc/host/pairs_dag.cpp
--- a/stem_kernel_amd/csrc/host/pairs_dag.cpp
+++ b/stem_kernel_amd/csrc/host/pairs_dag.cpp
@@ -402,7 +402,7 @@
     std::fprintf(stderr, "[phi] keys=%zu items=%zu item keys=%zu pairs=%lld phi components=%zu rows=%zu "
                  "classes=%zu sharing=%zu tables=%zu\n",
                  PX.phi_al.size(), plan.items.size(), item_phi.size(), (long long)n, PX.phk_idx.size(),
-                 PX.xgrow.size(), plan.classes.size(), shared, slots);
+                 PX.run_rows().size(), plan.classes.size(), shared, slots);
   }
 
   if (host_stats) th2 = now_ms();
@@ -487,8 +487,8 @@
     }
     const double gap2 = kp->loop_gap * kp->loop_gap;
     const size_t nnd = std::max<size_t>(PX.nd_a.size(), 1);
-    const size_t nxc = std::max<size_t>(PX.xr_ch.size(), 1), nxg = std::max<size_t>(PX.xgrow.size(), 1),
-                 nxgc = std::max<size_t>(PX.xg_ch.size(), 1),
+    const size_t nxc = std::max<size_t>(PX.xr_ch.size(), 1), nxg = std::max<size_t>(PX.run_rows().size(), 1),
+                 nxgc = std::max<size_t>(PX.run_ch().size(), 1),
                  ngh = std::max<size_t>(PX.ex_nl.size() * PX.gam_key.size(), 1),
                  nphk = std::max<size_t>(PX.phk_idx.size(), 1);
     if (!xs_->prep) {
diff --git a/stem_kernel_amd/csrc/host/runtime_types.h b/stem_kernel_amd/csrc/host/runtime_types.h
--- a/stem_kernel_amd/csrc/host/runtime_types.h
+++ b/stem_kernel_amd/csrc/host/runtime_types.h
@@ -105,9 +105,22 @@
   pvec<uint32_t> gra_gidx, gra_row, phk_idx;
   std::vector<int32_t> ex_gra_base, ex_phk_base;
   pvec<uint64_t> ex_phi_bits;
+  pvec<sk::XRow> xf_row;
+  pvec<uint32_t> xf_node, xf_ch, xf_clg, xf_gra_row;
+  pvec<float> xf_cpf;
+  pvec<uint8_t> xf_cty;
+  std::vector<int32_t> ex_xf_base, ex_nlxf, ex_xfch_base, ex_ss_rows, ex_ss_repl;
+  bool shared_sums = false;
   int32_t max_nl = 0, max_edges = 0, max_bpf = 0, max_nlev = 0, max_len = 0, max_slots = 0;
   int32_t max_nch = 0;
-};
+  const pvec<sk::XRow>& run_rows() const { return shared_sums ? xf_row : xgrow; }
+  const pvec<uint32_t>& run_ch() const { return shared_sums ? xf_ch : xg_ch; }
+  const std::vector<int32_t>& run_base() const { return shared_sums ? ex_xf_base : ex_xg_base; }
+  const std::vector<int32_t>& run_nl() const { return shared_sums ? ex_nlxf : ex_nlxg; }
+  const std::vector<int32_t>& run_ch_base() const { return shared_sums ? ex_xfch_base : ex_xgch_base; }
+};
+#define SK_PACK_F_ARRAYS(X) X(xf_row) X(xf_node) X(xf_ch) X(xf_clg) X(xf_cpf) X(xf_cty) X(xf_gra_row) \
+  X(ex_xf_base) X(ex_nlxf) X(ex_xfch_base) X(ex_ss_rows) X(ex_ss_repl)
 #define SK_PACK_Y_ARRAYS(X) X(yn_a) X(yn_b) X(yn_c) X(ye2) X(ysc) X(yrec) X(yn_w) X(yn_nbp) X(yn_p0) X(yn_P) \
   X(ycs) X(ex_ysc_base) X(ex_nch) X(ex_ycs_base)
 #define SK_PACK_X_ARRAYS(X) X(nd_a) X(nd_b) X(nd_c) X(nd_w) X(nd_nbp) X(nd_P) X(ed) X(bpf_code) X(bpf_p)     \
diff --git a/stem_kernel_amd/kernel_matrix.py b/stem_kernel_amd/kernel_matrix.py
--- a/stem_kernel_amd/kernel_matrix.py
+++ b/stem_kernel_amd/kernel_matrix.py
@@ -465,6 +465,11 @@
         return dict(zip(("rows", "stored", "slab_reads", "gamma_reads", "phi_reads", "reg_reads",
                          "y_slots"), (a.value for a in v)))
 
+    def shared_sums(self, i: int):
+        v = [C.c_int32() for _ in range(2)]
+        check(lib().sk_dataset_shared_sums(self._h, i, *[C.byref(a) for a in v]))
+        return v[0].value, v[1].value
+
     def dag(self, i: int) -> dict:
         nn, ne, nb, nr, L = self.shape(i)
         u = lambda k: np.zeros(max(k, 1), np.uint32)
```

New measurement: 249,200, median of 6. 1.09x the previous value.
